# zhan-xu/MoRig

Measured on AMD Instinct MI355X. Metric: meshes/sec jointnet_motion forward, 4 k-vert synthetic, higher is better.
Workload: dtype f32 (split-fp16: 3x f16 MFMA, f32 accumulate); 1 GPU; jointnet_motion(num_keyframes=5, attn) eval forward, B=64 x 4096-vertex synthetic meshes/GPU, BASELINE.json configs[1]; step=COO->CSR prep + forward, meshes_per_gpu=64, global_batch=64, vertices_per_mesh=4096, parallelism=mesh-sharded dp1, guard_read=deferred, geo_graph=device

## Files before the change

include/morig_hip.h:

```cpp
#ifndef MORIG_HIP_H
#define MORIG_HIP_H

#include <stdint.h>
#include <string.h>

#ifdef __cplusplus
extern "C" {
#endif

#define MORIG_ABI_VERSION 3

#define MORIG_INIT_ARGS(type, var) type var; memset(&(var), 0, sizeof(var)); (var).struct_size = (uint32_t)sizeof(var)
#define MORIG_GEMM_ARGS_V3_SIZE        192u
#define MORIG_EDGECONV_ARGS_V3_SIZE    192u
#define MORIG_EDGECONV_X3_ARGS_V3_SIZE 168u
#define MORIG_SEGMAX_ARGS_V3_SIZE      144u
#define MORIG_POINTCONV_ARGS_V3_SIZE   176u
#define MORIG_EDGECONV_ARGS_SIZE       216u
#define MORIG_EDGECONV_X3_ARGS_SIZE    184u

#define MORIG_OK              0
#define MORIG_E_INVALID      -1
#define MORIG_E_UNSUPPORTED  -2
#define MORIG_E_HIP          -3
#define MORIG_E_NODEVICE     -4

int         morig_abi_version(void);
int         morig_reserve_cus(int n);
const char* morig_strerror(int status);
int         morig_last_hip_error(void);
int         morig_device_info(int* cu_count, int* lds_bytes_per_cu, int* clock_khz, char* arch, int arch_len);

int morig_csr_build(const int64_t* edge_index, int64_t n_edges, int32_t n_nodes,
                    int32_t* rowptr, int32_t* src_sorted, int32_t* dst_sorted,
                    int32_t* cursor, int32_t* status, void* stream);
#define MORIG_CSR_SKIP_NEGATIVE 1
#define MORIG_CSR_PAD4          2
#define MORIG_CSR_MIN4          4
int morig_csr_build_bipartite(const int64_t* edge_index, int64_t n_edges, int32_t n_src_nodes, int32_t n_nodes,
                              int32_t flags, int32_t* rowptr, int32_t* src_sorted, int32_t* dst_sorted,
                              int32_t* cursor, int32_t* status, void* stream);

#define MORIG_SPLIT_F16 0
#define MORIG_SPLIT_BF16 1
#define MORIG_SPLIT_BF16X6 2
typedef struct morig_gemm_args {
    uint32_t struct_size;
    int32_t M, N, K;
    const float* X; int32_t ldx;
    const float* W; int32_t ldw;
    const float* bias;
    const float* scale;
    const float* shift;
    int32_t relu;
    const float* rowbias; int32_t ld_rowbias;
    const int32_t* seg;
    float* Y; int32_t ldy;
    float* pool; int32_t ld_pool; int32_t n_seg;
    const void* W_split; int32_t* overflow;
    int32_t x_split, y_split;
    int32_t w_split_format;
    const float* X_tail; int32_t ld_tail, tail_rows, tail_cols;
} morig_gemm_args;
int morig_gemm(const morig_gemm_args* a, void* stream);

typedef struct morig_edgeconv_args {
    uint32_t struct_size;
    int32_t H;
    int32_t n_nodes, replicas;
    int32_t in_rep_stride;
    int32_t out_rep_stride;
    const float* A; int32_t lda;
    const float* B; int32_t ldb;
    const int32_t* rowptr; const int32_t* src_sorted; const int32_t* dst_sorted;
    int32_t edge_capacity;
    int32_t edge_count;
    const float* s1; const float* t1;
    const float* W2; int32_t ldw;
    const float* b2; const float* s2; const float* t2;
    float* out; int32_t ldo;
    const void* W2_split; int32_t* overflow;
    int32_t quad_aligned;
    int32_t out_split;
    int32_t exact_arith;
    int32_t seg_min4;
    const struct morig_edgeconv_args* init_with;
    const struct morig_edgeconv_args* split_with;
    int32_t skip_init, skip_split;
} morig_edgeconv_args;
int morig_edgeconv(const morig_edgeconv_args* a, void* stream);
int morig_edgeconv_can_split_out(const morig_edgeconv_args* a);

typedef struct morig_edgeconv_x3_args {
    uint32_t struct_size;
    int32_t H;
    int32_t n_nodes, replicas;
    int32_t in_rep_stride, out_rep_stride;
    const float* X; int32_t ldx;
    const float* W1a; const float* W1b; const float* b1;
    const int32_t* rowptr; const int32_t* src_sorted; const int32_t* dst_sorted;
    int32_t edge_capacity; int32_t edge_count;
    const float* W2; int32_t ldw;
    const float* b2; const float* s2; const float* t2;
    float* out; int32_t ldo;
    const void* W2_split; int32_t* overflow;
    const struct morig_edgeconv_x3_args* init_with;
    int32_t skip_init, reserved0;
} morig_edgeconv_x3_args;
int morig_edgeconv_x3(const morig_edgeconv_x3_args* a, void* stream);

int morig_edge_hidden(const morig_edgeconv_args* a, void* stream);
typedef struct morig_segmax_args {
    uint32_t struct_size;
    int32_t N, K;
    const float* X; int32_t ldx;
    const float* W; int32_t ldw;
    const float* bias; const float* scale; const float* shift; int32_t relu;
    const int32_t* rowptr; const int32_t* dst_sorted; int32_t n_nodes;
    int32_t edge_capacity; int32_t edge_count;
    float* out; int32_t ldo;
    const void* W_split; int32_t* overflow;
} morig_segmax_args;
int morig_segmax_gemm(const morig_segmax_args* a, void* stream);

typedef struct morig_pointconv_args {
    uint32_t struct_size;
    const float* A; int32_t lda;
    const float* B; int32_t ldb;
    const int64_t* slots; int32_t max_nbrs;
    int32_t n_centres, n_src;
    int32_t H, H3;
    const void* W2_split; int32_t ldw2; const float* b2;
    const void* W3_split; int32_t ldw3; const float* b3; const float* s3; const float* t3; int32_t relu3;
    float* out; int32_t ldo;
    int32_t* overflow; int32_t* status;
} morig_pointconv_args;
int morig_pointconv_fused(const morig_pointconv_args* a, void* stream);

int morig_copy2d(const float* src, int32_t lds, float* dst, int32_t ldd, int32_t rows, int32_t cols, void* stream);
int morig_copy2d_pad(const float* src, int32_t lds, int32_t rows, int32_t cols, float* dst, int32_t ldd,
                     int32_t slot_cols, int32_t split, int32_t* overflow, void* stream);
int morig_copy2d_pad_rep(const float* src, int32_t lds, int32_t rows, int32_t cols, int32_t src_col_step, float* dst,
                         int32_t ldd, int32_t slot_cols, int32_t replicas, int64_t dst_row_step, int32_t split,
                         int32_t* overflow, void* stream);
#define MORIG_MAX_TAILS 8
int morig_pack_tails(const float* src, int32_t lds, int32_t rows, const int32_t* col_a ,
                     const int32_t* col_b , int32_t wa, int32_t wb, int32_t n_tails, float* dst,
                     int64_t tail_stride, int32_t* overflow, void* stream);

int morig_gather_cols(const float* src, int32_t lds, const int32_t* cols, int32_t n_cols,
                      float* dst, int32_t ldd, int32_t rows, void* stream);

int morig_make_seg(const int64_t* batch, int32_t n_nodes, int32_t n_graphs, int32_t replicas,
                   int32_t* seg_out, void* stream);

int morig_rownorm(const float* x, int32_t ldx, int32_t rows_per_rep, int32_t replicas, int32_t cols,
                  float* y, int32_t ld_row, int32_t ld_rep, void* stream);

int morig_cls_attention(const float* x, int32_t n, int32_t T, int32_t C, int32_t heads,
                        const float* g, const float* cls, float* y, int32_t ldy, void* stream);

int morig_frame_reduce(const float* x, int32_t n, int32_t T, int32_t C, int32_t mode, float* y, int32_t ldy, void* stream);

int morig_csr_build_dual(const int64_t* edge_index, int64_t n_edges, int32_t n_nodes, int32_t* rowptr, int32_t* src_sorted,
                         int32_t* dst_sorted, int32_t* rowptr4, int32_t* src_sorted4, int32_t* dst_sorted4, int32_t* ws,
                         int32_t flags, int32_t* status, void* stream);
int morig_csr_from_slots(const int64_t* coo, int32_t n_nodes, int32_t max_nbrs, int32_t n_src_nodes,
                         int32_t* rowptr, int32_t* src_sorted, int32_t* dst_sorted, int32_t* cursor, int32_t* status,
                         void* stream);
int morig_fps(const float* pos, int32_t ldp, const int32_t* ptr, const int32_t* out_ptr, const int32_t* start,
              int32_t n_clouds, int32_t max_cloud_points, int32_t* idx_out, void* stream);
int morig_ball_query(const float* x, int32_t ldx, const int32_t* ptr_x, const float* y, int32_t ldy,
                     const int32_t* ptr_y, int32_t n_clouds, int32_t n_centres, float radius,
                     int32_t max_nbrs, int64_t* coo, void* stream);
int morig_radius_sample(const float* x, int32_t ldx, int32_t nx, const float* y, int32_t ldy, int32_t ny, float radius,
                        int32_t max_nbrs, uint32_t seed, int64_t* coo, int32_t* counts, void* stream);
int morig_knn_interpolate(const float* feat, int32_t ldf, int32_t C, const float* pos_x, int32_t ldx,
                          const int32_t* ptr_x, const float* pos_y, int32_t ldy, const int32_t* ptr_y,
                          int32_t n_clouds, int32_t n_targets, int32_t max_targets_per_cloud, int32_t k,
                          int32_t* idx_ws, float* wgt_ws, float* out, int32_t ldo, void* stream);
int morig_knn_search(const float* pos_x, int32_t ldx, const int32_t* ptr_x, const float* pos_y, int32_t ldy,
                     const int32_t* ptr_y, int32_t n_clouds, int32_t n_targets, int32_t max_targets_per_cloud, int32_t k,
                     int32_t* idx, float* wgt, void* stream);
int morig_knn_apply(const float* feat, int32_t ldf, int32_t C, const int32_t* idx, const float* wgt, int32_t n_targets,
                    float* out, int32_t ldo, void* stream);
int morig_cosine_nn(const float* v, int32_t ldv, const int32_t* ptr_v, const float* p, int32_t ldp,
                    const int32_t* ptr_p, int32_t n_clouds, int32_t max_rows_per_cloud, int32_t C,
                    int32_t* nn, float* sim, void* stream);
int morig_sigmoid_minmax(const float* x, int32_t ldx, const int32_t* ptr, int32_t n_meshes, float* out, int32_t ldo,
                         void* stream);
int morig_cosine_knn(const float* y, int32_t ldy, const int32_t* ptr_y, const float* x, int32_t ldx,
                     const int32_t* ptr_x, int32_t n_clouds, int32_t max_rows_per_cloud, int32_t C, int32_t k,
                     const float* vis, int32_t ld_vis, int32_t split, int32_t* idx, void* stream);
int morig_flow_vote(int32_t mode, const int32_t* idx, int32_t k, int32_t n, const float* feat_q, int32_t ldq,
                    const float* feat_s, int32_t lds, int32_t C, const float* pos_q, int32_t ldpq,
                    const float* pos_s, int32_t ldps, const float* vis, int32_t ld_vis, float* l1, int32_t ld_l1,
                    void* stream);
int morig_inside_check(const double* pts, int32_t n, const uint8_t* vox88, const double* translate, double scale,
                       double dims0, uint8_t* keep, void* stream);
int morig_knn_bandwidth(const double* pts, int32_t n, int32_t k, double* kth_ws, double* bandwidth, void* stream);
int morig_meanshift(const double* pts, const float* weights, int32_t n, const double* bandwidth, int32_t max_iter,
                    double* buf_a, double* buf_b, double* state, int32_t* result_in_a, void* stream);
int morig_nms_counts(const double* pts, int32_t n, const double* bandwidth, int32_t* counts, void* stream);
int morig_nms_greedy(const double* pts, const float* attn, int32_t n, const double* bandwidth, const int32_t* order,
                     double thrd_density, float thrd_attn, uint8_t* alive, void* stream);
int morig_knn_bandwidth_batched(const double* pts, const int32_t* ptr, int32_t n_meshes, int32_t n_all, int32_t max_n,
                                double quantile, double* kth_ws, double* bandwidth, void* stream);
int morig_meanshift_batched(const double* pts, const float* weights, const int32_t* ptr, int32_t n_meshes, int32_t n_all,
                            int32_t max_n, const double* bandwidth, int32_t max_iter, double* buf_a, double* buf_b,
                            double* state, int32_t* result_in_a, void* stream);
int morig_nms_counts_batched(const double* pts, const int32_t* ptr, int32_t n_meshes, int32_t n_all, int32_t max_n,
                             const double* bandwidth, int32_t* counts, void* stream);
int morig_nms_greedy_batched(const double* pts, const float* attn, const int32_t* ptr, int32_t n_meshes, int32_t n_all,
                             const double* bandwidth, const int32_t* order_local, double thrd_density, float thrd_attn,
                             uint8_t* alive, void* stream);
int morig_morton_keys(const double* pts, const int32_t* ptr, int32_t n_meshes, int32_t n_all, int64_t* keys, void* stream);
int morig_nms_counts_sorted(const double* pts, const int32_t* ptr, int32_t n_meshes, int32_t n_all, int32_t max_n,
                            const double* bandwidth, double* bbox_ws, int32_t* counts, void* stream);
int morig_meanshift_sorted(const double* pts, const float* weights, const int32_t* ptr, int32_t n_meshes, int32_t n_all,
                           int32_t max_n, const double* bandwidth, int32_t max_iter, double* buf_a, double* buf_b,
                           double* state, double* bbox_ws, int32_t* result_in_a, void* stream);
int morig_gather_rows(const float* src, int32_t lds, const int32_t* idx, int32_t rows, int32_t cols,
                      float* dst, int32_t ldd, void* stream);

int morig_geo_ball_graph(const float* pos, int32_t ldp, const int32_t* mesh_ptr, int32_t n_meshes, int32_t n_nodes,
                         float radius, int32_t max_nn, uint32_t seed, int32_t* slots, int32_t* counts, int32_t* members,
                         int32_t* offsets, int32_t* scan_ws, void* stream);
int morig_geo_ball_graph_dist(const double* dist, int64_t ldd, int32_t n_nodes, double radius, int32_t max_nn, uint32_t seed,
                              int32_t* slots, int32_t* counts, int32_t* members, int32_t* offsets, int32_t* scan_ws,
                              void* stream);
int morig_geo_ball_fill(const int32_t* slots, const int32_t* offsets, int32_t n_nodes, int32_t max_nn, int32_t self_loops,
                        int64_t* coo, int64_t n_out, void* stream);

int64_t morig_vol_geodesic_workspace(int32_t n_meshes, int32_t n_slots);
int morig_vol_geodesic(const uint8_t* vox, int32_t n_meshes, const double* vox_tf, const double* pos, const int32_t* vtx_ptr,
                       const double* bones, const int32_t* bone_ptr, int32_t n_jobs, const int64_t* dist_off, int32_t n_slots,
                       void* workspace, int64_t workspace_bytes, int32_t* status, int32_t* dist, void* stream);
int morig_skin_bind(const int32_t* dist, const int64_t* dist_off, const int32_t* vtx_ptr, const int32_t* bone_ptr, int32_t n_meshes,
                    int32_t n_vertices, const double* bones, const uint8_t* is_leaf, const int32_t* start_jid, const double* skins,
                    int32_t ld_skins, int32_t k, int32_t* bind_ids, double* bind_invd, double* labels, float* skin_input,
                    int64_t* skin_nn, int64_t* loss_mask, int64_t* skin_nnjids, void* stream);
int morig_skin_scatter(const float* logits, int32_t ldl, const int64_t* skin_nn, const int64_t* loss_mask, const int64_t* batch,
                       const int32_t* n_bones, int32_t n, int32_t k, int32_t mode, double* P, int32_t ldp, void* stream);
int morig_skin_filter(const double* P, int32_t ldp, const int32_t* rowptr, const int32_t* cols, const int64_t* batch,
                      const int32_t* n_bones, int32_t n, double ratio, double* W, int32_t ldw, void* stream);

int64_t morig_surface_geodesic_workspace(int64_t total_samples, int32_t n_meshes, int32_t max_samples, int32_t n_slots, int32_t use_lds);
int morig_surface_geodesic(const double* pts, const double* normals, const int32_t* s_ptr, const int32_t* job_ptr, int32_t n_meshes,
                           int64_t total_samples, int32_t max_samples, int32_t n_jobs, int32_t nsrc, int32_t use_lds,
                           const int64_t* out_off, int32_t n_slots, void* workspace, int64_t workspace_bytes, int32_t* status,
                           double* out, void* stream);
int morig_nearest_point(const double* q, const int32_t* q_ptr, const double* pts, const int32_t* p_ptr, int32_t n_meshes, int32_t n_q,
                        int32_t squared, int32_t* out, void* stream);
int morig_bone_point_distance(const double* pos, const int32_t* vtx_ptr, const double* bones, const int32_t* bone_ptr, int32_t n_meshes,
                              const int64_t* off, int64_t n_pairs, double* origins, double* dist, void* stream);
int morig_bone_visibility(const double* pos, const int32_t* vtx_ptr, const double* bones, const int32_t* bone_ptr, const double* tri_pos,
                          const int32_t* tp_ptr, const int32_t* faces, const int32_t* f_ptr, const int64_t* off, const int32_t* blk_ptr,
                          int32_t n_meshes, int32_t n_blocks, uint8_t* vis, void* stream);
int morig_bone_geodesic(const double* dist, const uint8_t* vis, const double* sg, const int64_t* sg_off, const int32_t* vtx_ptr,
                        const int32_t* bone_ptr, const int64_t* off, int32_t n_meshes, int32_t n_bones, int64_t n_pairs,
                        uint8_t* vis_after, int32_t* n_vis, double* pct, double* out, int32_t* nn, void* stream);
// ... 363 lines not shown
```

morig_amd/csrc/common.h:

```cpp
#pragma once
#include <hip/hip_runtime.h>
#include <stdint.h>
#include <string.h>
#include "../../include/morig_hip.h"
#include "ragged_core.h"
#include "mfma_types.h"
#include "launch_core.h"

namespace morig {

constexpr float FP16_RANGE_GUARD = 65000.f;

enum Kind : int {
    K_GEMM_BN128 = 0, K_GEMM_BN64, K_GEMM_BN32, K_GEMM_POOL,
    K_EDGE_H16, K_EDGE_H32, K_EDGE_H64, K_EDGE_H128, K_EDGE_H256,
    K_CSR, K_COPY, K_ROWNORM, K_ATTN, K_MISC,
    K_FPS, K_BALL, K_POINTCONV, K_KNN_INTERP, K_COSINE_NN,
    K_GEMM16_BN128, K_GEMM16_BN64, K_GEMM16_BN32, K_GEMM16_POOL,
    K_EDGE16_H32, K_EDGE16_H64, K_EDGE16_H128, K_EDGE16_H256, K_POINTCONV16, K_GEMM16_DMA,
    K_COSINE_KNN, K_FLOW_VOTE, K_JOINTS,
    K_GEMM16_DMAP, K_GEMM16_DMA128, K_EDGE16_H256_PP, K_EDGE16_H128_WS, K_EDGE16_PC, K_GEOGRAPH, K_EDGE16_X3, K_EDGE_X3, K_EDGE16_X3P, K_EDGE16_H128_RL,
    K_LOSS_NCE_FWD, K_LOSS_NCE_BWD, K_LOSS_MULTIPOS, K_LOSS_CHAMFER, K_LOSS_REDUCE,
    K_LOSS_LOGRATIO, K_LOSS_SKIN_CE,
    K_METRICS,
    K_RIG_ASSEMBLE, K_RIG_ENTRIES,
    K_RANSAC_VOTE, K_RANSAC_FIT, K_RANSAC_APPLY, K_KMEANS,
    K_MESH_PREP, K_VOXEL_SURFACE, K_VOXEL_FILL,
    K_POSE_PREP, K_POSE_SKIN, K_POSE_ERRORS,
    K_SCAN_RASTER, K_SCAN,
    K_SIMPLIFY_KEYS, K_SIMPLIFY_QUADRICS,
    K_RAY_CAST, K_RAY_SELECT, K_RAY_ATTENTION,
    K_TRANSFER_PAIRS, K_TRANSFER_FLOOD, K_TRANSFER_ROWS,
    K_BVH_BUILD, K_BVH_QUERY,
    K_COUNT
};
static_assert(K_COUNT <= MORIG_PROF_KINDS, "raise MORIG_PROF_KINDS");

void set_hip_error(hipError_t e);
struct ProfScope {
    ProfScope(int kind, hipStream_t s, double flops, double bytes);
    ~ProfScope();
    int slot; hipStream_t stream; ProfScope* outer;
};
void prof_retag(int kind);

inline int check_hip(hipError_t e) {
    if (e == hipSuccess) return MORIG_OK;
    set_hip_error(e);
    return MORIG_E_HIP;
}
#define MORIG_HIP_TRY(expr) do { hipError_t _e = (expr); if (_e != hipSuccess) { ::morig::set_hip_error(_e); return MORIG_E_HIP; } } while (0)
#define MORIG_LAUNCH_CHECK() MORIG_HIP_TRY(hipGetLastError())

struct EdgePcParams {
    int H;
    const float* W; int ldw;
    const float* bias; const float* scale; const float* shift;
    const float* A; int lda; const float* B; int ldb;
    const int* rowptr; const int* srcS; const int* dstS; int n_nodes; int rep_in; int rep_out; int tiles_per_rep;
    int replicas;
    float* Y; int ldy;
    int y16;
    int run;
    int* ovf;
    int quad;
    int min4;
    unsigned long long* trace;
    int dbg;
};
struct GemmDmaParams {
    int M, N, K;
    const float* X; int ldx;
    const float* Xt; int ldt; int tail_rows; int tail_chunks;
    const float* W; int ldw;
    const float* bias; const float* scale; const float* shift; int relu;
    const float* rowbias; int ld_rowbias; const int* seg;
    float* Y; int ldy; int y16;
    float* pool; int ld_pool;
    int tiles_n;
    int run;
    int* ovf;
    int dbg;
    unsigned long long* trace;
};
int launch_edge_pc(const EdgePcParams& p, int nblocks, hipStream_t s);
int launch_edge_pp(const EdgePcParams& p, int nblocks, hipStream_t s);
int launch_edge_ws(const EdgePcParams& p, int nblocks, hipStream_t s);
int launch_edge_rl(const EdgePcParams& p, int ntiles64, hipStream_t s);
int launch_gemm16_dma(const GemmDmaParams& p, int tiles_m128, hipStream_t s);
struct EdgeX3Params {
    const float* X; int ldx;
    const float* W1a; const float* W1b; const float* b1;
    const float* A; int lda; const float* B; int ldb;
    const float* W2s; int ldw;
    const float* bias; const float* scale; const float* shift;
    const int* rowptr; const int* srcS; const int* dstS; int n_nodes; int cap;
    int rep_in, rep_out, replicas;
    float* Y; int ldy;
    int* ovf;
};

int launch_edge_x3(const EdgeX3Params& p, int n_tiles_cap, hipStream_t s);
int launch_gemm16_dmap(const GemmDmaParams& p, hipStream_t s);
bool few_rows_gemm_takes(int M, int N, int K, int ldx, int ldw);
int launch_few_rows_gemm(const float* X, int ldx, int M, const float* W, int ldw, int N, int K, const float* bias, const float* scale,
                         const float* shift, int relu, float* Y, int ldy, hipStream_t s);

static_assert(sizeof(morig_gemm_args) >= MORIG_GEMM_ARGS_V3_SIZE && sizeof(morig_edgeconv_args) >= MORIG_EDGECONV_ARGS_V3_SIZE &&
              sizeof(morig_edgeconv_x3_args) >= MORIG_EDGECONV_X3_ARGS_V3_SIZE && sizeof(morig_segmax_args) >= MORIG_SEGMAX_ARGS_V3_SIZE &&
              sizeof(morig_pointconv_args) >= MORIG_POINTCONV_ARGS_V3_SIZE, "argument structs only grow");
static_assert(sizeof(morig_edgeconv_args) == MORIG_EDGECONV_ARGS_SIZE && sizeof(morig_edgeconv_x3_args) == MORIG_EDGECONV_X3_ARGS_SIZE,
              "include/morig_hip.h states the current sizes");
template <class T> static inline bool take_args(const T* a, T& mine, uint32_t v3_size) {
    if (!a) return false;
    const uint32_t n = a->struct_size;
    if (n < v3_size || n > 1024u || (n & 7u)) return false;
    memset(&mine, 0, sizeof(T));
    memcpy(&mine, a, n < sizeof(T) ? n : sizeof(T));
    mine.struct_size = (uint32_t)sizeof(T);
    return true;
}

static inline int cdiv(long a, long b) { return (int)((a + b - 1) / b); }

__device__ __forceinline__ void atomic_max_f32(float* addr, float v) {
    if (v == 0.0f) v = 0.0f;
    if (v >= 0.0f) atomicMax(reinterpret_cast<int*>(addr), __float_as_int(v));
    else           atomicMin(reinterpret_cast<unsigned int*>(addr), __float_as_uint(v));
}

__device__ __forceinline__ int xcd_remap(int b, int n) {
    const int q = n >> 3, r = n & 7, x = b & 7, i = b >> 3;
    return (x < r ? x * (q + 1) : r * (q + 1) + (x - r) * q) + i;
}

inline int stats_slab_rows(int rows_cap, int cols) {
    const int groups = (cols + 63) / 64;
    int slabs = 1024 / (groups > 0 ? groups : 1);
    if (slabs < 64) slabs = 64;
    int r = ((rows_cap > 0 ? rows_cap : 1) + slabs - 1) / slabs;
    r = (r + 3) & ~3;
    return r < 256 ? 256 : r;
}

#ifdef __HIPCC__
__device__ inline void split_pair_f16(float v0, float v1, float& hi, float& lo) {
    typedef __fp16 split_h2 __attribute__((ext_vector_type(2)));
    const split_h2 h = __builtin_amdgcn_cvt_pkrtz(v0, v1);
    hi = __builtin_bit_cast(float, h);
#ifdef MORIG_SPLIT_C_FORM
    split_h2 l;
    l[0] = (__fp16)(v0 - (float)h[0]); l[1] = (__fp16)(v1 - (float)h[1]);
    lo = __builtin_bit_cast(float, l);
#else
    asm("v_fma_mixlo_f16 %0, %1, 1.0, -%2 op_sel_hi:[0,0,1]" : "=v"(lo) : "v"(v0), "v"(hi));
    asm("v_fma_mixhi_f16 %0, %1, 1.0, -%2 op_sel:[0,0,1] op_sel_hi:[0,0,1]" : "+v"(lo) : "v"(v1), "v"(hi));
#endif
}
#endif

#ifdef __HIPCC__
__device__ inline void split_pair_bf16(float v0, float v1, float& hi, float& lo) {
    typedef __bf16 split_b2 __attribute__((ext_vector_type(2)));
    const split_b2 h = {(__bf16)v0, (__bf16)v1};
    const unsigned hb = __builtin_bit_cast(unsigned, h);
    hi = __builtin_bit_cast(float, h);
    const float r0 = v0 - __uint_as_float(hb << 16), r1 = v1 - __uint_as_float(hb & 0xffff0000u);
    const split_b2 l = {(__bf16)r0, (__bf16)r1};
    lo = __builtin_bit_cast(float, l);
}
#endif

#ifdef __HIPCC__
__device__ inline void split_pair_bf16_rem(float v0, float v1, float& hi, float& r0, float& r1) {
    typedef __bf16 split_b2 __attribute__((ext_vector_type(2)));
    const split_b2 h = {(__bf16)v0, (__bf16)v1};
    const unsigned hb = __builtin_bit_cast(unsigned, h);
    hi = __builtin_bit_cast(float, h);
    r0 = v0 - __uint_as_float(hb << 16);
    r1 = v1 - __uint_as_float(hb & 0xffff0000u);
}
#endif

template <int V> struct VecF { float v[V]; };
#ifdef __HIPCC__
template <int V> __device__ inline VecF<V> ldv(const float* p) {
    VecF<V> r;
    if constexpr (V == 4) { const float4 t = *reinterpret_cast<const float4*>(p); r.v[0] = t.x; r.v[1] = t.y; r.v[2] = t.z; r.v[3] = t.w; }
    else r.v[0] = *p;
    return r;
}
template <int V> __device__ inline void stv(float* p, const VecF<V>& r) {
    if constexpr (V == 4) *reinterpret_cast<float4*>(p) = make_float4(r.v[0], r.v[1], r.v[2], r.v[3]);
    else *p = r.v[0];
}
#endif
static inline bool vec4_ptr(const void* p, long ld) { return (reinterpret_cast<uintptr_t>(p) & 15) == 0 && (ld & 3) == 0; }

#ifdef __HIPCC__
__device__ inline void stats_block_store(const double (&acc)[2][4], int quads, int RL, int q, int rl, int c0, int cols, int slab,
                                         double* __restrict__ part) {
    __shared__ double sh[2 * 1024];
    const int gc = quads * 4;
    if (rl < RL) {
#pragma unroll
        for (int k = 0; k < 2; ++k)
#pragma unroll
            for (int j = 0; j < 4; ++j) sh[(k * gc + q * 4 + j) * RL + rl] = acc[k][j];
    }
    __syncthreads();
    const int t = threadIdx.x;
    if (t < 2 * gc) {
        const int k = t / gc, col = t - k * gc;
        double s = 0.0;
        for (int i = 0; i < RL; ++i) s += sh[(k * gc + col) * RL + i];
        if (c0 + col < cols) part[((size_t)slab * 2 + k) * cols + c0 + col] = s;
    }
}

constexpr int STATS_FC = 4;
__device__ inline void stats_final_sums(const double* __restrict__ part, int slabs, int cols, int c, double& s, double& q) {
    const int sl = threadIdx.x / STATS_FC, l = threadIdx.x % STATS_FC;
    constexpr int LANES = 256 / STATS_FC;
    s = 0.0; q = 0.0;
    if (c < cols)
        for (int b = sl; b < slabs; b += LANES) { s += part[((size_t)b * 2 + 0) * cols + c]; q += part[((size_t)b * 2 + 1) * cols + c]; }
    __shared__ double sh[2][LANES][STATS_FC];
    sh[0][sl][l] = s; sh[1][sl][l] = q;
    __syncthreads();
    for (int h = LANES / 2; h > 0; h >>= 1) {
        if (sl < h) { sh[0][sl][l] += sh[0][sl + h][l]; sh[1][sl][l] += sh[1][sl + h][l]; }
        __syncthreads();
    }
    s = sh[0][0][l]; q = sh[1][0][l];
}

__device__ __forceinline__ double block_sum256(double s, double* sh) {
    sh[threadIdx.x] = s;
    __syncthreads();
    for (int h = 128; h > 0; h >>= 1) {
        if ((int)threadIdx.x < h) sh[threadIdx.x] += sh[threadIdx.x + h];
        __syncthreads();
    }
    const double r = sh[0];
    __syncthreads();
    return r;
}
#endif

}
```

morig_amd/csrc/edge_x3.hip:

```cpp
#include "common.h"

namespace morig {


constexpr int X3_BM = 128, X3_LINE = 144;

template <bool AB>
__global__ __launch_bounds__(256, 4) void edge_x3_kernel(const EdgeX3Params p) {
    __shared__ __attribute__((aligned(16))) char lines[2][X3_BM * X3_LINE];
    __shared__ int sseg[2][X3_BM];
    __shared__ int sstart[2][X3_BM + 2];
    __shared__ int snseg[2];
    __shared__ int sflag[2][2];

    const int tid = threadIdx.x, lane = tid & 63, wave = tid >> 6;
    const int l31 = lane & 31, hi = lane >> 5;
    const int row = wave * 32 + l31;
    const int Etot = p.rowptr[p.n_nodes];
    const int tpr = (Etot + X3_BM - 1) / X3_BM;
    const int T = tpr * p.replicas;
    if ((int)blockIdx.x >= T) return;

    f16x8 w1h, w1l, wh[2], wl[2];
    {
        float v[8] = {0.f, 0.f, 0.f, 0.f, 0.f, 0.f, 0.f, 0.f};
        if (!AB && hi == 0) {
#pragma unroll
            for (int j = 0; j < 3; ++j) { v[j] = p.W1a[l31 * 4 + j]; v[3 + j] = p.W1b[l31 * 4 + j]; }
            v[6] = p.b1[l31];
        }
        f32x4 hb, lb;
#pragma unroll
        for (int q = 0; q < 4; ++q) { float h2, l2; split_pair_f16(v[2 * q], v[2 * q + 1], h2, l2); hb[q] = h2; lb[q] = l2; }
        w1h = __builtin_bit_cast(f16x8, hb); w1l = __builtin_bit_cast(f16x8, lb);
        const char* wr = reinterpret_cast<const char*>(p.W2s + (size_t)l31 * p.ldw);
#pragma unroll
        for (int st = 0; st < 2; ++st) {
            wh[st] = *reinterpret_cast<const f16x8*>(wr + 32 * st + 16 * hi);
            wl[st] = *reinterpret_cast<const f16x8*>(wr + 64 + 32 * st + 16 * hi);
        }
    }
    const float cb = p.bias[l31], cs = p.scale[l31], ct = p.shift[l31];

    auto tile_row0 = [&](int t, int& rep) __attribute__((always_inline)) { rep = t / tpr; return (t - rep * tpr) * X3_BM; };
    auto load_ids = [&](int t, int& d, int& sidx, int& edge) __attribute__((always_inline)) {
        if (t >= T) return;
        int rep; const int r0 = tile_row0(t, rep);
        const int r = min(r0 + row, Etot - 1);
        d = p.dstS[r]; sidx = p.srcS[r];
        if (tid < 2) edge = p.dstS[min(max(tid == 0 ? r0 - 1 : r0 + X3_BM, 0), Etot - 1)];
    };
    auto load_x = [&](int t, int d, int sidx, f32x4& a, f32x4& b) __attribute__((always_inline)) {
        if (AB || t >= T || hi != 0) return;
        int rep; const int r0 = tile_row0(t, rep);
        const bool live = r0 + row < Etot;
        const size_t base = (size_t)rep * p.rep_in;
        a = *reinterpret_cast<const f32x4*>(p.X + (base + (live ? d : 0)) * p.ldx);
        b = *reinterpret_cast<const f32x4*>(p.X + (base + (live ? sidx : 0)) * p.ldx);
    };
    auto load_ab = [&](int t, int d, int sidx, f32x4 (&a)[4], f32x4 (&b)[4]) __attribute__((always_inline)) {
        if (!AB || t >= T) return;
        int rep; const int r0 = tile_row0(t, rep);
        const bool live = r0 + row < Etot;
        const size_t base = (size_t)rep * p.rep_in;
        const float* ar = p.A + (base + (live ? d : 0)) * p.lda + 4 * hi;
        const float* br = p.B + (base + (live ? sidx : 0)) * p.ldb + 4 * hi;
#pragma unroll
        for (int g4 = 0; g4 < 4; ++g4) { a[g4] = *reinterpret_cast<const f32x4*>(ar + 8 * g4); b[g4] = *reinterpret_cast<const f32x4*>(br + 8 * g4); }
    };
    const int t0 = blockIdx.x, tstep = gridDim.x;
    int d_cur = 0, s_cur = 0, e_cur = 0, d_nxt = 0, s_nxt = 0, e_nxt = 0;
    f32x4 xi_cur = {0.f, 0.f, 0.f, 0.f}, xj_cur = xi_cur, xi_nxt = xi_cur, xj_nxt = xi_cur;
    f32x4 ga_cur[4], gb_cur[4], ga_nxt[4], gb_nxt[4];
#pragma unroll
    for (int g4 = 0; g4 < 4; ++g4) ga_cur[g4] = gb_cur[g4] = ga_nxt[g4] = gb_nxt[g4] = xi_cur;
    load_ids(t0, d_cur, s_cur, e_cur);
    load_ids(t0 + tstep, d_nxt, s_nxt, e_nxt);
    load_x(t0, d_cur, s_cur, xi_cur, xj_cur);
    load_ab(t0, d_cur, s_cur, ga_cur, gb_cur);
    bool amax_bad = false;

    int par = 0;
    for (int t = t0; t < T; t += tstep, par ^= 1) {
        int rep; const int r0 = tile_row0(t, rep);
        const bool live = r0 + row < Etot;
        load_x(t + tstep, d_nxt, s_nxt, xi_nxt, xj_nxt);
        load_ab(t + tstep, d_nxt, s_nxt, ga_nxt, gb_nxt);
        int d_nn = 0, s_nn = 0, e_nn = 0;
        load_ids(t + 2 * tstep, d_nn, s_nn, e_nn);

        char* L = lines[par];
        if (hi == 0) sseg[par][row] = live ? d_cur : -1;
        if (tid == 0) sflag[par][0] = (r0 > 0 && d_cur == e_cur) ? 1 : 0;
        {
            f32x16 a1;
            if constexpr (AB) {
#pragma unroll
                for (int g4 = 0; g4 < 4; ++g4)
#pragma unroll
                    for (int q = 0; q < 4; ++q) a1[4 * g4 + q] = ga_cur[g4][q] + gb_cur[g4][q];
            } else {
                f32x4 hb = {0.f, 0.f, 0.f, 0.f}, lb = hb;
                if (hi == 0) {
                    float h2, l2;
                    split_pair_f16(xi_cur[0], xi_cur[1], h2, l2); hb[0] = h2; lb[0] = l2;
                    split_pair_f16(xi_cur[2], xj_cur[0], h2, l2); hb[1] = h2; lb[1] = l2;
                    split_pair_f16(xj_cur[1], xj_cur[2], h2, l2); hb[2] = h2; lb[2] = l2;
                    split_pair_f16(1.0f, 0.0f, h2, l2);           hb[3] = h2; lb[3] = l2;
                    const float am = fmaxf(fmaxf(fmaxf(fabsf(xi_cur[0]), fabsf(xi_cur[1])), fmaxf(fabsf(xi_cur[2]), fabsf(xj_cur[0]))),
                                           fmaxf(fabsf(xj_cur[1]), fabsf(xj_cur[2])));
                    if (!(am < FP16_RANGE_GUARD)) amax_bad = true;
                }
                const f16x8 xh = __builtin_bit_cast(f16x8, hb), xl = __builtin_bit_cast(f16x8, lb);
#pragma unroll
                for (int r = 0; r < 16; ++r) a1[r] = 0.f;
                a1 = __builtin_amdgcn_mfma_f32_32x32x16_f16(w1l, xh, a1, 0, 0, 0);
                a1 = __builtin_amdgcn_mfma_f32_32x32x16_f16(w1h, xl, a1, 0, 0, 0);
                a1 = __builtin_amdgcn_mfma_f32_32x32x16_f16(w1h, xh, a1, 0, 0, 0);
            }
            char* line = L + row * X3_LINE;
            float am = 0.f, chk = 0.f;
#pragma unroll
            for (int g4 = 0; g4 < 4; ++g4) {
                float h[4];
#pragma unroll
                for (int q = 0; q < 4; ++q) {
                    if (AB) chk = fmaf(a1[4 * g4 + q], 0.f, chk);
                    h[q] = fmaxf(a1[4 * g4 + q], 0.f); am = fmaxf(am, h[q]);
                }
                float h0, l0, h1, l1;
                split_pair_f16(h[0], h[1], h0, l0);
                split_pair_f16(h[2], h[3], h1, l1);
                typedef float f32x2 __attribute__((ext_vector_type(2)));
                const f32x2 hv = {h0, h1}, lv = {l0, l1};
                const int c0 = 8 * g4 + 4 * hi;
                *reinterpret_cast<f32x2*>(line + 2 * c0) = hv;
                *reinterpret_cast<f32x2*>(line + 64 + 2 * c0) = lv;
            }
            if (!(chk == 0.f) || !(am < FP16_RANGE_GUARD)) amax_bad = true;
        }
        asm volatile("" ::: "memory");
        f32x16 acc;
#pragma unroll
        for (int r = 0; r < 16; ++r) acc[r] = 0.f;
        {
            const char* ar = L + (wave * 32 + l31) * X3_LINE + 16 * hi;
#pragma unroll
            for (int st = 0; st < 2; ++st) {
                const f16x8 ah = *reinterpret_cast<const f16x8*>(ar + 32 * st);
                const f16x8 al = *reinterpret_cast<const f16x8*>(ar + 64 + 32 * st);
                acc = __builtin_amdgcn_mfma_f32_32x32x16_f16(al, wh[st], acc, 0, 0, 0);
                acc = __builtin_amdgcn_mfma_f32_32x32x16_f16(ah, wl[st], acc, 0, 0, 0);
                acc = __builtin_amdgcn_mfma_f32_32x32x16_f16(ah, wh[st], acc, 0, 0, 0);
            }
        }
        asm volatile("" ::: "memory");
        {
            float* Z = reinterpret_cast<float*>(L);
#pragma unroll
            for (int r = 0; r < 16; ++r) {
                const int rl = wave * 32 + (r & 3) + 8 * (r >> 2) + 4 * hi;
                Z[rl * (X3_LINE / 4) + l31] = fmaxf(acc[r] + cb, 0.f) * cs + ct;
            }
        }
        __syncthreads();
        if (wave == 0) {
            const int rA = lane, rB = lane + 64;
            const bool f0 = rA == 0 || sseg[par][rA] != sseg[par][rA - 1];
            const bool f1 = sseg[par][rB] != sseg[par][rB - 1];
            const unsigned long long m0 = __ballot(f0), m1 = __ballot(f1);
            const unsigned long long below = (1ull << lane) - 1ull;
            if (f0) sstart[par][__popcll(m0 & below)] = rA;
            if (f1) sstart[par][__popcll(m0) + __popcll(m1 & below)] = rB;
            if (lane == 0) { const int ns = __popcll(m0) + __popcll(m1); snseg[par] = ns; sstart[par][ns] = X3_BM; }
            if (lane == 1) sflag[par][1] = (r0 + X3_BM < Etot && sseg[par][X3_BM - 1] == e_cur) ? 1 : 0;
        }
        __syncthreads();
        {
            const float* Z = reinterpret_cast<const float*>(L);
            const int c4 = (tid & 7) * 4, slot = tid >> 3;
            const int nseg = snseg[par];
            const bool first_cont = sflag[par][0] != 0, last_cont = sflag[par][1] != 0;
            float* obase = p.Y + (size_t)rep * p.rep_out * p.ldy + c4;
            for (int k = slot; k < nseg; k += 32) {
                const int rs = sstart[par][k], re = sstart[par][k + 1];
                const int sg = sseg[par][rs];
                if (sg < 0) continue;
                f32x4 m = *reinterpret_cast<const f32x4*>(Z + rs * (X3_LINE / 4) + c4);
                for (int r = rs + 1; r < re; r += 4) {
                    f32x4 z[4];
#pragma unroll
                    for (int u = 0; u < 4; ++u) z[u] = *reinterpret_cast<const f32x4*>(Z + min(r + u, re - 1) * (X3_LINE / 4) + c4);
#pragma unroll
                    for (int u = 0; u < 4; ++u)
#pragma unroll
                        for (int q = 0; q < 4; ++q) m[q] = fmaxf(m[q], z[u][q]);
                }
                float* o = obase + (size_t)sg * p.ldy;
                const bool partial = (rs == 0 && first_cont) || (re == X3_BM && last_cont);
                if (partial) {
#pragma unroll
                    for (int q = 0; q < 4; ++q) atomic_max_f32(o + q, m[q]);
                } else {
                    *reinterpret_cast<f32x4*>(o) = m;
                }
            }
        }
        d_cur = d_nxt; s_cur = s_nxt; e_cur = e_nxt; xi_cur = xi_nxt; xj_cur = xj_nxt;
        if constexpr (AB) {
#pragma unroll
            for (int g4 = 0; g4 < 4; ++g4) { ga_cur[g4] = ga_nxt[g4]; gb_cur[g4] = gb_nxt[g4]; }
        }
        d_nxt = d_nn; s_nxt = s_nn; e_nxt = e_nn;
    }
    if (amax_bad) *p.ovf = 1;
}

int launch_edge_x3(const EdgeX3Params& p, int n_tiles_cap, hipStream_t s) {
    int avail = cu_count() - reserved_cus();
    if (avail < 8) avail = 8;
    int grid = avail * 4;
    if (grid > n_tiles_cap) grid = n_tiles_cap;
    if (grid < 1) grid = 1;
    if (p.X) hipLaunchKernelGGL(edge_x3_kernel<false>, dim3(grid), dim3(256), 0, s, p);
    else     hipLaunchKernelGGL(edge_x3_kernel<true>, dim3(grid), dim3(256), 0, s, p);
    MORIG_LAUNCH_CHECK();
    return MORIG_OK;
}

}
```

morig_amd/csrc/prof.hip:

```cpp
#include "common.h"
#include <atomic>
#include <mutex>
#include <stdlib.h>
#include <vector>
#include <string.h>

namespace morig {

static int g_last_hip = 0;
void set_hip_error(hipError_t e) { g_last_hip = (int)e; }

int cu_count() {
    static std::atomic<int> cache[64];
    int dev = 0;
    if (hipGetDevice(&dev) != hipSuccess || dev < 0 || dev >= 64) return 256;
    int n = cache[dev].load();
    if (n == 0) {
        if (hipDeviceGetAttribute(&n, hipDeviceAttributeMultiprocessorCount, dev) != hipSuccess || n <= 0) n = 256;
        cache[dev].store(n);
    }
    return n;
}

static std::atomic<int> g_reserved_cus{0};
void set_reserved_cus(int n) { g_reserved_cus.store(n < 0 ? 0 : n); }
int reserved_cus() { return g_reserved_cus.load(); }

int persistent_grid(int units) {
    int ncu = cu_count();
    ncu = ncu > 8 ? (ncu / 8) * 8 : 8;
    int avail = ncu - ((reserved_cus() + 7) / 8) * 8;
    if (avail < 8) avail = 8;
    return units < avail ? ((units + 7) / 8) * 8 : avail;
}

int debug_flags() {
    static const int v = [] { const char* e = getenv("MORIG_DEBUG_FLAGS"); return e ? atoi(e) : 0; }();
    return v;
}

struct Slot { hipEvent_t a, b; int kind; double flops, bytes; };
static std::mutex g_mu;
static bool g_on = false;
static std::vector<Slot> g_slots;
static std::vector<Slot> g_free;
static double g_ms[K_COUNT], g_fl[K_COUNT], g_by[K_COUNT];
static long long g_n[K_COUNT];

static thread_local ProfScope* t_scope = nullptr;

ProfScope::ProfScope(int kind, hipStream_t s, double flops, double bytes) : slot(-1), stream(s), outer(t_scope) {
    t_scope = this;
    std::lock_guard<std::mutex> lk(g_mu);
    if (!g_on) return;
    Slot sl;
    if (!g_free.empty()) { sl = g_free.back(); g_free.pop_back(); }
    else {
        if (hipEventCreate(&sl.a) != hipSuccess) return;
        if (hipEventCreate(&sl.b) != hipSuccess) { (void)hipEventDestroy(sl.a); return; }
    }
    sl.kind = kind; sl.flops = flops; sl.bytes = bytes;
    (void)hipEventRecord(sl.a, s);
    g_slots.push_back(sl);
    slot = (int)g_slots.size() - 1;
}
ProfScope::~ProfScope() {
    t_scope = outer;
    if (slot < 0) return;
    std::lock_guard<std::mutex> lk(g_mu);
    if (slot < (int)g_slots.size()) (void)hipEventRecord(g_slots[slot].b, stream);
}

void prof_retag(int kind) {
    ProfScope* p = t_scope;
    if (!p || p->slot < 0) return;
    std::lock_guard<std::mutex> lk(g_mu);
    if (p->slot < (int)g_slots.size()) g_slots[p->slot].kind = kind;
}

static void drain_locked() {
    for (auto& s : g_slots) {
        float ms = 0.f;
        if (hipEventSynchronize(s.b) == hipSuccess && hipEventElapsedTime(&ms, s.a, s.b) == hipSuccess) {
            g_ms[s.kind] += ms; g_fl[s.kind] += s.flops; g_by[s.kind] += s.bytes; g_n[s.kind] += 1;
        }
        g_free.push_back(s);
    }
    g_slots.clear();
}

static const char* kNames[K_COUNT] = {
    "gemm_f32_bn128", "gemm_f32_bn64", "gemm_f32_bn32", "gemm_f32_pool",
    "edgeconv_h16", "edgeconv_h32", "edgeconv_h64", "edgeconv_h128", "edgeconv_h256",
    "csr_build", "copy", "rownorm", "cls_attention", "misc",
    "fps", "ball_query", "pointconv", "knn_interpolate", "cosine_nn",
    "gemm_f16x3_bn128", "gemm_f16x3_bn64", "gemm_f16x3_bn32", "gemm_f16x3_pool",
    "edgeconv_f16x3_h32", "edgeconv_f16x3_h64", "edgeconv_f16x3_h128", "edgeconv_f16x3_h256", "pointconv_f16x3", "gemm_f16x3_dma",
    "cosine_knn", "flow_vote", "joint_extraction",
    "gemm_f16x3_dmap", "gemm_f16x3_dma128", "edgeconv_f16x3_h256_pp", "edgeconv_f16x3_h128_ws", "edgeconv_f16x3_pc", "geo_graph", "edgeconv_f16x3_x3", "edgeconv_x3", "edgeconv_f16x3_x3_persistent", "edgeconv_f16x3_h128_rl",
    "loss_infonce_fwd", "loss_infonce_bwd", "loss_multipos", "loss_chamfer", "loss_reduce",
    "loss_logratio", "loss_skin_ce",
    "rig_metrics",
    "rig_assemble", "rig_skin_entries",
    "ransac_vote", "ransac_fit", "ransac_apply", "kernel_kmeans",
    "mesh_prep", "voxel_surface", "voxel_fill",
    "pose_prep", "pose_skin", "pose_traj_errors",
    "scan_raster", "scan",
    "simplify_keys", "simplify_quadrics",
    "ray_cast", "ray_select", "ray_attention",
    "transfer_pairs", "transfer_flood", "transfer_rows",
    "bvh_build", "bvh_query",
};
static const char* kSymbols[K_COUNT] = {
    "tile_kernel<128, 32, 0, 0, 0,", "tile_kernel<64, 32, 0, 0, 0,", "tile_kernel<32, 32, 0, 0, 0,", "tile_kernel<128, 32, 0, 1, 0,",
    "tile_kernel<32, 16, 1, 2, 0,", "tile_kernel<32, 32, 1, 2, 0,", "tile_kernel<64, 32, 1, 2, 0,", "tile_kernel<128, 32, 1, 2, 0,", "tile_kernel<256, 16, 1, 2, 0,",
    nullptr, nullptr, "rownorm", "cls_attention_kernel", nullptr,
    nullptr, nullptr, nullptr, nullptr, nullptr,
    "tile_kernel<128, 32, 0, 0, 1,", "tile_kernel<64, 32, 0, 0, 1,", "tile_kernel<32, 32, 0, 0, 1,", "gemm16_dmap_kernel<true>",
    "tile_kernel<32, 32, 1, 2, 1,", "tile_kernel<64, 32, 1, 2, 1,", "edge_pp_kernel<128", "edge_ws_kernel<256", nullptr, "gemm16_dma_kernel<256, 256, 4, 2",
    nullptr, nullptr, nullptr,
    "gemm16_dmap_kernel<false>", "gemm16_dma_kernel<128, 128, 2, 2", "edge_pp_kernel<256", "edge_ws_kernel<128", "edge_pc_kernel", "geo_ball_graph_kernel", "tile_kernel<32, 32, 2, 2, 1,", "tile_kernel<32, 32, 2, 2, 0,", "edge_x3_kernel", "edge_rl128_kernel",
    "nce_fwd_kernel", "nce_bwd_kernel", nullptr, nullptr, nullptr,
    nullptr, nullptr,
    nullptr,
    "rig_assemble_kernel", nullptr,
    "ransac_vote_kernel", "ransac_fit_kernel", "ransac_apply_kernel", "kmeans_kernel",
    nullptr, "voxel_surface_kernel", "voxel_fill_kernel",
    nullptr, "pose_skin_kernel", "pose_errors_kernel",
    nullptr, nullptr,
    nullptr, "simplify_quadrics_kernel",
    "ray_cast_kernel", "ray_select_kernel", "ray_attention_kernel",
    nullptr, nullptr, nullptr,
    nullptr, nullptr,
};

}

using namespace morig;

extern "C" {

int morig_abi_version(void) { return MORIG_ABI_VERSION; }

int morig_reserve_cus(int n) { set_reserved_cus(n); return MORIG_OK; }

const char* morig_strerror(int st) {
    switch (st) {
        case MORIG_OK: return "ok";
        case MORIG_E_INVALID: return "invalid argument (null pointer, negative size or misaligned leading dimension)";
        case MORIG_E_UNSUPPORTED: return "unsupported width/shape for the instantiated gfx950 kernels";
        case MORIG_E_HIP: return "HIP runtime error (see morig_last_hip_error)";
        case MORIG_E_NODEVICE: return "no gfx950 device visible";
        default: return "unknown status";
    }
}

int morig_last_hip_error(void) { return g_last_hip; }

int morig_device_info(int* cu_count, int* lds_bytes_per_cu, int* clock_khz, char* arch, int arch_len) {
    int n = 0;
    if (hipGetDeviceCount(&n) != hipSuccess || n <= 0) return MORIG_E_NODEVICE;
    int dev = 0;
    MORIG_HIP_TRY(hipGetDevice(&dev));
    hipDeviceProp_t p;
    MORIG_HIP_TRY(hipGetDeviceProperties(&p, dev));
    if (cu_count) *cu_count = p.multiProcessorCount;
    if (lds_bytes_per_cu) *lds_bytes_per_cu = (int)p.maxSharedMemoryPerMultiProcessor;
    if (clock_khz) *clock_khz = p.clockRate;
    if (arch && arch_len > 0) { strncpy(arch, p.gcnArchName, arch_len - 1); arch[arch_len - 1] = 0; }
    return strncmp(p.gcnArchName, "gfx950", 6) == 0 ? MORIG_OK : MORIG_E_NODEVICE;
}

int morig_prof_enable(int on) {
    std::lock_guard<std::mutex> lk(g_mu);
    int prev = g_on ? 1 : 0;
    g_on = on != 0;
    return prev;
}

int morig_prof_reset(void) {
    std::lock_guard<std::mutex> lk(g_mu);
    drain_locked();
    for (int k = 0; k < K_COUNT; ++k) { g_ms[k] = g_fl[k] = g_by[k] = 0.0; g_n[k] = 0; }
    return MORIG_OK;
}

const char* morig_prof_name(int kind) { return (kind >= 0 && kind < K_COUNT) ? kNames[kind] : nullptr; }
const char* morig_prof_symbol(int kind) { return (kind >= 0 && kind < K_COUNT) ? kSymbols[kind] : nullptr; }

int morig_prof_collect(int kind, int64_t* launches, double* total_ms, double* flops, double* bytes) {
    if (kind < 0 || kind >= K_COUNT) return MORIG_E_INVALID;
    std::lock_guard<std::mutex> lk(g_mu);
    drain_locked();
    if (launches) *launches = g_n[kind];
    if (total_ms) *total_ms = g_ms[kind];
    if (flops) *flops = g_fl[kind];
    if (bytes) *bytes = g_by[kind];
    return MORIG_OK;
}

}
```

morig_amd/csrc/tile_gemm.hip:

```cpp
#include "common.h"
#include "epilogue_store.h"
#include <stdint.h>
#include <stdlib.h>
#include <type_traits>

namespace morig {

typedef _Float16 f16x4 __attribute__((ext_vector_type(4)));
typedef __fp16 f16x2 __attribute__((ext_vector_type(2)));

enum { PREC_F32 = 0, PREC_F16X3 = 1, PREC_BF16X3 = 2, PREC_BF16X6 = 3 };

enum { LOAD_DENSE = 0, LOAD_EDGE = 1, LOAD_EDGE3 = 2 };
enum { MODE_STORE = 0, MODE_POOL = 1, MODE_EDGEMAX = 2 };

struct TileParams {
    int M, N, K;
    const float* W; int ldw;
    const float* bias; const float* scale; const float* shift; int relu;
    const float* X; int ldx;
    const float* A; int lda; const float* B; int ldb;
    const float* X3; int ldx3; const float* W1a; const float* W1b; const float* b1;
    const int* rowptr; const int* srcS; const int* dstS; int n_nodes; int rep_in; int rep_out; int tiles_per_rep;
    const float* s1; const float* t1;
// ... 392 lines not shown
        }
        __syncthreads();
        const int c4 = (tid & 7) * 4, slot = tid >> 3;
        const int col0 = tn * BN + c4;
        if (col0 >= p.N) return;
        const int nseg = snseg;
        float* obase = p.Y + (size_t)rep * p.rep_out * p.ldy + col0;
        const bool vec_ok = (reinterpret_cast<uintptr_t>(p.Y) & 15) == 0 && (p.ldy & 3) == 0 && col0 + 4 <= p.N;
        for (int k = slot; k < nseg; k += 32) {
            const int rs = sstart[k], re = sstart[k + 1];
            const int sg = sseg[rs];
            if (sg < 0) continue;
            f32x4 m = *reinterpret_cast<const f32x4*>(Z + rs * ZL + c4);
            for (int r = rs + 1; r < re; r += 4) {
                f32x4 z[4];
#pragma unroll
                for (int u = 0; u < 4; ++u) z[u] = *reinterpret_cast<const f32x4*>(Z + min(r + u, re - 1) * ZL + c4);
#pragma unroll
                for (int u = 0; u < 4; ++u)
#pragma unroll
                    for (int q = 0; q < 4; ++q) m[q] = fmaxf(m[q], z[u][q]);
            }
            float* o = obase + (size_t)sg * p.ldy;
            const bool partial = (rs == 0 && first_cont) || (re == BM && last_cont);
            if (partial) {
#pragma unroll
                for (int q = 0; q < 4; ++q) if (col0 + q < p.N) atomic_max_f32(o + q, m[q]);
            } else if (vec_ok) {
                *reinterpret_cast<f32x4*>(o) = m;
            } else {
#pragma unroll
                for (int q = 0; q < 4; ++q) if (col0 + q < p.N) o[q] = m[q];
            }
        }
        return;
    }
    constexpr int NTP = ((ZC / 32) / WN) >= 1 ? ((ZC / 32) / WN) : 1;
    constexpr int NPASS = NT / NTP;
    static_assert(NTP * WN * 32 == ZC && NPASS * NTP == NT, "epilogue column blocking");
    constexpr int G = 256 / ZC;
    constexpr int RG = BM / G;
    const int zc = tid % ZC, zg = tid / ZC;
    const int r0 = (ZC == 64) ? __builtin_amdgcn_readfirstlane(zg * RG) : zg * RG;
    unsigned long long seg_start_lo = 0, seg_start_hi = 0, seg_own = 0; int seg_id_own = 0;
    if constexpr (MODE == MODE_EDGEMAX && ZC == 64) {
        const int s_lo = sseg[lane], s_hi = sseg[lane + 64];
        const int p_lo = sseg[lane > 0 ? lane - 1 : 0], p_hi = sseg[lane + 63];
        seg_start_lo = __ballot(lane == 0 || s_lo != p_lo); seg_start_hi = __ballot(s_hi != p_hi);
        const bool up = r0 >= 64;
        const unsigned long long valid = up ? __ballot(s_hi >= 0) : __ballot(s_lo >= 0);
        seg_own = (up ? seg_start_hi : seg_start_lo) & valid & (((1ull << RG) - 1ull) << (r0 & 63));
        seg_id_own = up ? s_hi : s_lo;
    }
    auto run_pass = [&](auto cb_const) {
        constexpr int cb = decltype(cb_const)::value;
        __syncthreads();
#pragma unroll
        for (int j = 0; j < NTP; ++j) {
            constexpr int dummy = 0; (void)dummy;
            const int nt = cb * NTP + j;
            const int col = tn * BN + wn * NT * 32 + nt * 32 + l31;
            const float b = (p.bias && col < p.N) ? p.bias[col] : 0.f;
            const float sc = (p.scale && col < p.N) ? p.scale[col] : 1.f;
            const float sh = (p.shift && col < p.N) ? p.shift[col] : 0.f;
#pragma unroll
            for (int mt = 0; mt < MT; ++mt)
#pragma unroll
                for (int r = 0; r < 16; ++r) {
                    const int rl = wm * MT * 32 + mt * 32 + (r & 3) + 8 * (r >> 2) + 4 * hi;
                    float v = acc[mt][nt][r] + b;
                    if (p.relu) v = v > 0.f ? v : 0.f;
                    Z[rl * ZLD + (wn * NTP + j) * 32 + l31] = v * sc + sh;
                }
        }
        __syncthreads();
        const int wz = zc / (NTP * 32), jz = (zc >> 5) % NTP;
        const int col = tn * BN + wz * NT * 32 + (cb * NTP + jz) * 32 + (zc & 31);
        if (col >= p.N) return;
        const float* zcolp = Z + zc;
        if (MODE == MODE_POOL) {
            int cur = -2; bool open = false; float m = 0.f;
#pragma unroll
            for (int bt = 0; bt < RG / 16; ++bt) {
                const int rb0 = r0 + bt * 16;
                float zv[16]; int sv[16];
#pragma unroll
                for (int i = 0; i < 16; ++i) {
                    sv[i] = (ZC == 64) ? __builtin_amdgcn_readfirstlane(sseg[rb0 + i]) : sseg[rb0 + i];
                    zv[i] = zcolp[(rb0 + i) * ZLD];
                }
#pragma unroll
                for (int i = 0; i < 16; ++i) {
                    if (sv[i] != cur) {
                        if (open) atomic_max_f32(p.Y + (size_t)cur * p.ldy + col, m);
                        cur = sv[i]; open = cur >= 0; m = zv[i];
                    } else if (open) m = fmaxf(m, zv[i]);
                }
            }
            if (open) atomic_max_f32(p.Y + (size_t)cur * p.ldy + col, m);
        } else {
            if constexpr (ZC == 64) {
            float* obase = p.Y + (size_t)rep * p.rep_out * p.ldy + col;
            const bool upper = r0 >= 64;
            unsigned long long mine = seg_own;
            while (mine) {
                const int bl = __builtin_ctzll(mine);
                mine &= mine - 1ull;
                const unsigned long long above = bl < 63 ? ~((2ull << bl) - 1ull) : 0ull;
                int rs, re;
                if (upper) {
                    const unsigned long long later = seg_start_hi & above;
                    rs = 64 + bl; re = later ? 64 + __builtin_ctzll(later) : BM;
                } else {
                    const unsigned long long later = seg_start_lo & above;
                    rs = bl; re = later ? __builtin_ctzll(later) : (seg_start_hi ? 64 + __builtin_ctzll(seg_start_hi) : BM);
                }
                const int sg = __builtin_amdgcn_readlane(seg_id_own, bl);
                float m = zcolp[rs * ZLD];
                for (int r = rs + 1; r < re; r += 4) {
                    const int l = re - 1;
                    const float z0 = zcolp[r * ZLD], z1 = zcolp[min(r + 1, l) * ZLD], z2 = zcolp[min(r + 2, l) * ZLD], z3 = zcolp[min(r + 3, l) * ZLD];
                    m = fmaxf(fmaxf(m, z0), fmaxf(fmaxf(z1, z2), z3));
                }
                float* o = obase + (size_t)sg * p.ldy;
                if ((rs == 0 && first_cont) || (re == BM && last_cont)) atomic_max_f32(o, m); else *o = m;
            }
            }
        }
    };
    run_pass(std::integral_constant<int, 0>{});
    if constexpr (NPASS > 1) run_pass(std::integral_constant<int, 1>{});
    if constexpr (NPASS > 2) run_pass(std::integral_constant<int, 2>{});
    if constexpr (NPASS > 3) run_pass(std::integral_constant<int, 3>{});
    static_assert(NPASS <= 4, "column passes");
}

__device__ __forceinline__ int straddled_row(const int* __restrict__ rowptr, const int* __restrict__ dstS, int n_nodes, int tile_rows,
                                             int run, int replicas, int rep_out, int g, int n_cand, bool last_only) {
    if (g > n_cand) return -1;
    const int Etot = rowptr[n_nodes];
    const int tpr = (Etot + tile_rows - 1) / tile_rows;
    if (tpr <= 0) return -1;
    const long long t = (long long)g * run;
    const int rep = (int)(t / tpr), tile = (int)(t - (long long)rep * tpr);
    if (rep >= replicas || tile == 0) return -1;
    const int e = tile * tile_rows;
    const int d = dstS[e];
    if (rowptr[d] >= e) return -1;
    if (last_only && (long long)e + (long long)run * tile_rows < rowptr[d + 1]) return -1;
    return rep * rep_out + d;
}

struct BoundaryJob { const int* rowptr; const int* dstS; int n_nodes, H; float* out; int ldo, rep_out, tile_rows, run, replicas, n_cand; int* ovf; };
struct BoundaryJobs { BoundaryJob j[2]; };

__global__ __launch_bounds__(256) void init_boundary_rows_kernel(const BoundaryJobs js) {
    const BoundaryJob& b = js.j[blockIdx.y];
    if ((int)blockIdx.x * 256 >= b.n_cand) return;
    const int* __restrict__ rowptr = b.rowptr; const int* __restrict__ dstS = b.dstS;
    float* __restrict__ out = b.out;
    const int H = b.H, ldo = b.ldo;
    const int lane = threadIdx.x & 63;
    const int d = straddled_row(rowptr, dstS, b.n_nodes, b.tile_rows, b.run, b.replicas, b.rep_out, blockIdx.x * 256 + threadIdx.x + 1, b.n_cand, false);
    const bool vec = ((reinterpret_cast<uintptr_t>(out) | (uintptr_t)(ldo * 4) | (uintptr_t)(H * 4)) & 15) == 0;
    typedef unsigned u32x4 __attribute__((ext_vector_type(4)));
    unsigned long long todo = __ballot(d >= 0);
    while (todo) {
        const int l = __builtin_ctzll(todo);
        todo &= todo - 1;
        float* orow = out + (size_t)__builtin_amdgcn_readlane(d, l) * ldo;
        if (vec) {
            u32x4* o4 = reinterpret_cast<u32x4*>(orow);
            for (int c = lane; c < H / 4; c += 64) o4[c] = u32x4{0xFFFFFFFFu, 0xFFFFFFFFu, 0xFFFFFFFFu, 0xFFFFFFFFu};
        } else {
            unsigned* o = reinterpret_cast<unsigned*>(orow);
            for (int c = lane; c < H; c += 64) o[c] = 0xFFFFFFFFu;
        }
    }
}

static BoundaryJob boundary_job(const int* rowptr, const int* dstS, int n_nodes, int edge_capacity, int H, float* out, int ldo, int rep_out,
                                int slots, int tile_rows, int run, int* ovf) {
    BoundaryJob b = {};
    b.rowptr = rowptr; b.dstS = dstS; b.n_nodes = n_nodes; b.H = H; b.out = out; b.ldo = ldo; b.rep_out = rep_out;
    b.tile_rows = tile_rows; b.run = run; b.replicas = slots; b.ovf = ovf;
    const int n_cand = cdiv((long)cdiv(edge_capacity, tile_rows) * slots, run) - 1;
    b.n_cand = n_cand > 0 ? n_cand : 0;
    return b;
}

static int init_boundary_rows(const BoundaryJob* jobs, int n, hipStream_t s) {
    BoundaryJobs js = {};
    int m = 0, most = 0;
    for (int i = 0; i < n; ++i) if (jobs[i].n_cand > 0) { js.j[m++] = jobs[i]; most = jobs[i].n_cand > most ? jobs[i].n_cand : most; }
    if (m == 0) return MORIG_OK;
    hipLaunchKernelGGL(init_boundary_rows_kernel, dim3(cdiv(most, 256), m), dim3(256), 0, s, js);
    MORIG_LAUNCH_CHECK();
    return MORIG_OK;
}

static int init_boundary_rows(const int* rowptr, const int* dstS, int n_nodes, int edge_capacity, int H, float* out, int ldo,
                              int rep_out, int slots, hipStream_t s, int tile_rows = 128, int run = 1) {
    const BoundaryJob b = boundary_job(rowptr, dstS, n_nodes, edge_capacity, H, out, ldo, rep_out, slots, tile_rows, run, nullptr);
    return init_boundary_rows(&b, 1, s);
}

__global__ __launch_bounds__(256) void split_boundary_rows_kernel(const BoundaryJobs js) {
    const BoundaryJob& b = js.j[blockIdx.y];
    if ((int)blockIdx.x * 64 >= b.n_cand) return;
    const int* __restrict__ rowptr = b.rowptr; const int* __restrict__ dstS = b.dstS;
    float* __restrict__ out = b.out;
    int* __restrict__ ovf = b.ovf;
    const int H = b.H, ldo = b.ldo;
    const int lane = threadIdx.x & 63;
    const int g = (blockIdx.x * 4 + (threadIdx.x >> 6)) * 16 + lane + 1;
    const int d = lane < 16 ? straddled_row(rowptr, dstS, b.n_nodes, b.tile_rows, b.run, b.replicas, b.rep_out, g, b.n_cand, true) : -1;
    unsigned long long todo = __ballot(d >= 0);
    float am = 0.f;
    bool bad = false;
    while (todo) {
        int dr[4];
#pragma unroll
        for (int i = 0; i < 4; ++i) {
            const int l = todo ? __builtin_ctzll(todo) : -1;
            todo &= todo - 1;
            dr[i] = l >= 0 ? __builtin_amdgcn_readlane(d, l) : -1;
        }
        for (int c0 = 0; c0 < H; c0 += 256) {
            const int c = c0 + 4 * lane;
            float4 v[4];
#pragma unroll
            for (int i = 0; i < 4; ++i)
                if (dr[i] >= 0 && c < H) v[i] = *reinterpret_cast<const float4*>(out + (size_t)dr[i] * ldo + c);
#pragma unroll
            for (int i = 0; i < 4; ++i)
                if (dr[i] >= 0 && c < H) {
                    float h0, l0, h1, l1;
                    split_pair_f16(v[i].x, v[i].y, h0, l0);
                    split_pair_f16(v[i].z, v[i].w, h1, l1);
                    am = fmaxf(am, fmaxf(fmaxf(fabsf(v[i].x), fabsf(v[i].y)), fmaxf(fabsf(v[i].z), fabsf(v[i].w))));
                    bad |= !(v[i].x == v[i].x && v[i].y == v[i].y && v[i].z == v[i].z && v[i].w == v[i].w);
                    char* oc = reinterpret_cast<char*>(out + (size_t)dr[i] * ldo) + (c >> 5) * 128 + (c & 31) * 2;
                    *reinterpret_cast<float2*>(oc) = make_float2(h0, h1);
                    *reinterpret_cast<float2*>(oc + 64) = make_float2(l0, l1);
                }
        }
    }
    if (bad || !(am < FP16_RANGE_GUARD)) *ovf = 1;
}

static int split_boundary_rows(const BoundaryJob* jobs, int n, hipStream_t s) {
    BoundaryJobs js = {};
    int m = 0, most = 0;
    for (int i = 0; i < n; ++i) if (jobs[i].n_cand > 0) { js.j[m++] = jobs[i]; most = jobs[i].n_cand > most ? jobs[i].n_cand : most; }
    if (m == 0) return MORIG_OK;
    hipLaunchKernelGGL(split_boundary_rows_kernel, dim3(cdiv(most, 64), m), dim3(256), 0, s, js);
    MORIG_LAUNCH_CHECK();
    return MORIG_OK;
}

template <int BN, int KC, int LOAD, int MODE, int PREC = PREC_F32>
static int launch_tile(const TileParams& p0, int nblocks, hipStream_t s) {
    TileParams p = p0;
    p.dbg = debug_flags();
    if constexpr (BN == 128 && KC == 32 && LOAD == LOAD_DENSE && MODE == MODE_STORE) {
        static const bool no_fast = getenv("MORIG_TILE_NO_FAST") != nullptr;
        if (p.dbg == 0 && !no_fast && p.M % 128 == 0 && p.K % KC == 0) {
            hipLaunchKernelGGL((tile_kernel<BN, KC, LOAD, MODE, PREC, true>), dim3(nblocks), dim3(256), 0, s, p);
            MORIG_LAUNCH_CHECK();
            return MORIG_OK;
        }
    }
    hipLaunchKernelGGL((tile_kernel<BN, KC, LOAD, MODE, PREC>), dim3(nblocks), dim3(256), 0, s, p);
    MORIG_LAUNCH_CHECK();
    return MORIG_OK;
}

static inline bool aligned16(const void* p) { return (reinterpret_cast<uintptr_t>(p) & 15) == 0; }

__global__ void pool_identity_to_zero_kernel(float* __restrict__ pool, int64_t n) {
    const int64_t stride = (int64_t)gridDim.x * blockDim.x;
    unsigned* u = reinterpret_cast<unsigned*>(pool);
    for (int64_t i = (int64_t)blockIdx.x * blockDim.x + threadIdx.x; i < n; i += stride) if (u[i] == 0xFFFFFFFFu) u[i] = 0u;
}
static int pool_finalize(float* pool, int n_seg, int ld_pool, hipStream_t s) {
    const int64_t n = (int64_t)n_seg * ld_pool;
    int64_t blocks = (n + 255) / 256;
    if (blocks > 1024) blocks = 1024;
    hipLaunchKernelGGL(pool_identity_to_zero_kernel, dim3((int)blocks), dim3(256), 0, s, pool, n);
    MORIG_LAUNCH_CHECK();
    return MORIG_OK;
}

}

using namespace morig;

extern "C" int morig_gemm(const morig_gemm_args* a_in, void* stream) {
    morig_gemm_args mine;
    if (!take_args(a_in, mine, MORIG_GEMM_ARGS_V3_SIZE)) return MORIG_E_INVALID;
    const morig_gemm_args* a = &mine;
    if (!a->X || !a->W) return MORIG_E_INVALID;
    if (a->M < 0 || a->N <= 0 || a->K <= 0) return MORIG_E_INVALID;
    if (a->M == 0) return MORIG_OK;
    if ((a->ldx & 3) || (a->ldw & 3) || !aligned16(a->X) || !aligned16(a->W)) return MORIG_E_INVALID;
    const bool tail = a->X_tail != nullptr;
    if (tail) {
        if (!a->x_split || !a->W_split || a->tail_cols <= 0 || (a->tail_cols & 31) || (a->K & 31) || a->K <= a->tail_cols || a->tail_rows <= 0 ||
            (a->ld_tail & 31) || a->ld_tail < a->tail_cols || (reinterpret_cast<uintptr_t>(a->X_tail) & 127) ||
            (double)a->tail_rows * a->ld_tail * 4.0 >= 4.0e9) return MORIG_E_INVALID;
    }
    if (a->ldx < (((a->K - (tail ? a->tail_cols : 0)) + 3) & ~3) || a->ldw < ((a->K + 31) & ~31)) return MORIG_E_INVALID;
    const bool pool = a->pool != nullptr;
    if (tail && pool) return MORIG_E_UNSUPPORTED;
    if (!pool && !a->Y) return MORIG_E_INVALID;
    if (pool && a->Y) return MORIG_E_UNSUPPORTED;
    if ((pool || a->rowbias) && !a->seg) return MORIG_E_INVALID;
    hipStream_t s = reinterpret_cast<hipStream_t>(stream);

    TileParams p = {};
    p.M = a->M; p.N = a->N; p.K = a->K;
    p.W = a->W; p.ldw = a->ldw;
    p.bias = a->bias; p.scale = a->scale; p.shift = a->shift; p.relu = a->relu;
    p.X = a->X; p.ldx = a->ldx;
    p.rowbias = a->rowbias; p.ld_rowbias = a->ld_rowbias; p.seg = a->seg;
    const int tiles_m = cdiv(a->M, 128);
    const double flops = 2.0 * a->M * (double)a->N * a->K;
    const double bytes = 4.0 * ((double)a->M * a->K + (double)a->N * a->K + (pool ? 0.0 : (double)a->M * a->N));

    const bool x6 = a->W_split == nullptr && a->w_split_format == MORIG_SPLIT_BF16X6;
    if (x6 && (a->x_split || a->y_split)) return MORIG_E_INVALID;
    const bool f16 = a->W_split != nullptr;
    if (f16 && a->w_split_format != MORIG_SPLIT_F16 && a->w_split_format != MORIG_SPLIT_BF16) return MORIG_E_INVALID;
    const bool bf16 = f16 && a->w_split_format == MORIG_SPLIT_BF16;
    if (f16 && !bf16 && a->overflow == nullptr) return MORIG_E_INVALID;
    if (f16) {
        if (!aligned16(a->W_split)) return MORIG_E_INVALID;
        if (bf16 && (pool || a->x_split || a->y_split)) return MORIG_E_UNSUPPORTED;
        p.W = static_cast<const float*>(a->W_split); p.ovf = a->overflow;
    }
    const bool kc64 = f16 && a->K >= 64 && (a->ldw & 63) == 0 && a->ldw >= ((a->K + 63) & ~63) && !getenv("MORIG_KC32");
    if (a->x_split || a->y_split) {
        if (!f16) return MORIG_E_INVALID;
        if (a->x_split && ((a->ldx & 31) || a->ldx < (((a->K - (tail ? a->tail_cols : 0)) + 31) & ~31) || (reinterpret_cast<uintptr_t>(a->X) & 127))) return MORIG_E_INVALID;
        if (a->y_split && (pool || (a->ldy & 31) || (reinterpret_cast<uintptr_t>(a->Y) & 127))) return MORIG_E_INVALID;
        p.x16 = a->x_split ? 1 : 0; p.y16 = a->y_split ? 1 : 0;
    }
    if (pool) {
        if (a->n_seg <= 0 || a->ld_pool < a->N) return MORIG_E_INVALID;
        MORIG_HIP_TRY(hipMemsetAsync(a->pool, 0xFF, (size_t)a->n_seg * a->ld_pool * sizeof(float), s));
        if (f16 && a->x_split && a->N > 64 && !getenv("MORIG_NO_DMA")) {
            GemmDmaParams q = {};
            q.M = a->M; q.N = a->N; q.K = a->K; q.X = a->X; q.ldx = a->ldx; q.W = p.W; q.ldw = p.ldw;
            q.bias = a->bias; q.scale = a->scale; q.shift = a->shift; q.relu = a->relu; q.seg = a->seg;
            q.pool = a->pool; q.ld_pool = a->ld_pool; q.ovf = a->overflow;
            ProfScope ps(K_GEMM16_POOL, s, flops, bytes);
            const int st = launch_gemm16_dma(q, tiles_m, s);
            return st != MORIG_OK ? st : pool_finalize(a->pool, a->n_seg, a->ld_pool, s);
        }
        p.Y = a->pool; p.ldy = a->ld_pool;
        p.tiles_n = cdiv(a->N, 128);
        ProfScope ps(f16 ? K_GEMM16_POOL : K_GEMM_POOL, s, flops, bytes);
        int st;
        if (x6) st = launch_tile<128, 32, LOAD_DENSE, MODE_POOL, PREC_BF16X6>(p, tiles_m * p.tiles_n, s);
        else if (f16 && kc64 && getenv("MORIG_KC64")) st = launch_tile<128, 64, LOAD_DENSE, MODE_POOL, PREC_F16X3>(p, tiles_m * p.tiles_n, s);
        else st = f16 ? launch_tile<128, 32, LOAD_DENSE, MODE_POOL, PREC_F16X3>(p, tiles_m * p.tiles_n, s)
                      : launch_tile<128, 32, LOAD_DENSE, MODE_POOL>(p, tiles_m * p.tiles_n, s);
        return st != MORIG_OK ? st : pool_finalize(a->pool, a->n_seg, a->ld_pool, s);
    }
    p.Y = a->Y; p.ldy = a->ldy;
    if (f16 && a->x_split && a->N > 64 && !getenv("MORIG_NO_DMA")) {
        GemmDmaParams q = {};
        q.M = a->M; q.N = a->N; q.K = a->K; q.X = a->X; q.ldx = a->ldx; q.W = p.W; q.ldw = p.ldw;
        q.bias = a->bias; q.scale = a->scale; q.shift = a->shift; q.relu = a->relu;
        q.rowbias = a->rowbias; q.ld_rowbias = a->ld_rowbias; q.seg = a->seg;
        q.Y = a->Y; q.ldy = a->ldy; q.y16 = a->y_split ? 1 : 0; q.tiles_n = cdiv(a->N, 128); q.ovf = a->overflow;
        if (tail) { q.Xt = a->X_tail; q.ldt = a->ld_tail; q.tail_rows = a->tail_rows; q.tail_chunks = a->tail_cols / 32; }
        ProfScope ps(K_GEMM16_DMA, s, flops, bytes);
        return launch_gemm16_dma(q, tiles_m, s);
    }
    if (tail) return MORIG_E_UNSUPPORTED;
    if (!bf16 && !a->rowbias && !a->x_split && !a->y_split && few_rows_gemm_takes(a->M, a->N, a->K, a->ldx, a->ldw)) {
        ProfScope ps(K_MISC, s, flops, bytes);
        return launch_few_rows_gemm(a->X, a->ldx, a->M, a->W, a->ldw, a->N, a->K, a->bias, a->scale, a->shift, a->relu, a->Y, a->ldy, s);
    }
    if (bf16) {
        ProfScope ps(K_MISC, s, flops, bytes);
        if (a->N > 64) { p.tiles_n = cdiv(a->N, 128); return launch_tile<128, 32, LOAD_DENSE, MODE_STORE, PREC_BF16X3>(p, tiles_m * p.tiles_n, s); }
        p.tiles_n = 1;
        if (a->N > 32) return launch_tile<64, 32, LOAD_DENSE, MODE_STORE, PREC_BF16X3>(p, tiles_m, s);
        return launch_tile<32, 32, LOAD_DENSE, MODE_STORE, PREC_BF16X3>(p, tiles_m, s);
    }
    if (x6) {
        ProfScope ps(a->N > 64 ? K_GEMM_BN128 : (a->N > 32 ? K_GEMM_BN64 : K_GEMM_BN32), s, flops, bytes);
        if (a->N > 64) { p.tiles_n = cdiv(a->N, 128); return launch_tile<128, 32, LOAD_DENSE, MODE_STORE, PREC_BF16X6>(p, tiles_m * p.tiles_n, s); }
        p.tiles_n = 1;
        if (a->N > 32) return launch_tile<64, 32, LOAD_DENSE, MODE_STORE, PREC_BF16X6>(p, tiles_m, s);
        return launch_tile<32, 32, LOAD_DENSE, MODE_STORE, PREC_BF16X6>(p, tiles_m, s);
    }
    if (a->N > 64) {
        p.tiles_n = cdiv(a->N, 128);
        ProfScope ps(f16 ? K_GEMM16_BN128 : K_GEMM_BN128, s, flops, bytes);
        static const bool want64 = getenv("MORIG_KC64") != nullptr;
        if (f16 && kc64 && want64) return launch_tile<128, 64, LOAD_DENSE, MODE_STORE, PREC_F16X3>(p, tiles_m * p.tiles_n, s);
        return f16 ? launch_tile<128, 32, LOAD_DENSE, MODE_STORE, PREC_F16X3>(p, tiles_m * p.tiles_n, s)
                   : launch_tile<128, 32, LOAD_DENSE, MODE_STORE>(p, tiles_m * p.tiles_n, s);
// ... 126 lines not shown
    static const bool want_mix = [] { const char* e = getenv("MORIG_EDGE_MIX"); return !(e && e[0] == '0'); }();
    pl.mix = pl.wide && !one_shot && !want_pp && pl.pp_ok && !a->quad_aligned && a->seg_min4 && a->H == 256 && want_mix &&
             (a->lda & 3) == 0 && (a->ldb & 3) == 0;
    pl.use_ws = (quad_ok && !pl.use_rl && (a->H == 256 || ws128)) || (pl.mix && a->out_split);
    pl.tile_rows = ((pl.use_ws && a->H == 256) || pl.use_rl) ? 64 : 128;
    static const int run_env = [] { const char* e = getenv("MORIG_EDGE_RUN"); const int v = e ? atoi(e) : 8; return v < 1 ? 1 : (v > 4096 ? 4096 : v); }();
    pl.run = 1;
    if (pl.use_rl || (pl.use_ws && a->out_split)) {
        const long tiles = (long)cdiv(a->edge_capacity, pl.tile_rows) * a->replicas;
        const long units = pl.use_rl ? 2048 : 256;
        while (pl.run * 2 <= run_env && tiles / (units * 16) >= pl.run * 2) pl.run *= 2;
    }
    static const bool no_split = [] { const char* e = getenv("MORIG_EDGE_SPLIT_OUT"); return e && e[0] == '0'; }();
    pl.split_ok = (pl.use_rl || pl.use_ws || pl.mix) && !no_split && a->overflow != nullptr && (a->ldo & 31) == 0 &&
                  (reinterpret_cast<uintptr_t>(a->out) & 127) == 0;
    return pl;
}

extern "C" int morig_edgeconv_can_split_out(const morig_edgeconv_args* a_in) {
    morig_edgeconv_args mine;
    if (!take_args(a_in, mine, MORIG_EDGECONV_ARGS_V3_SIZE)) return 0;
    const morig_edgeconv_args* a = &mine;
    TileParams p = {};
    if (edge_common(a, p) != MORIG_OK) return 0;
    return edge_plan(a).split_ok ? 1 : 0;
}

extern "C" int morig_edgeconv(const morig_edgeconv_args* a_in, void* stream) {
    morig_edgeconv_args mine;
    if (!take_args(a_in, mine, MORIG_EDGECONV_ARGS_V3_SIZE)) return MORIG_E_INVALID;
    const morig_edgeconv_args* a = &mine;
    TileParams p = {};
    const int st = edge_common(a, p);
    if (st != MORIG_OK) return st;
    if (a->in_rep_stride < 0 || (a->replicas > 1 && a->out_rep_stride < a->n_nodes)) return MORIG_E_INVALID;
    hipStream_t s = reinterpret_cast<hipStream_t>(stream);
    const int nblocks = p.tiles_per_rep * a->replicas;
    const bool f16 = a->W2_split != nullptr;
    const EdgePlan pl = edge_plan(a);
    const bool wide = pl.wide, one_shot = pl.one_shot, pp_ok = pl.pp_ok, use_rl = pl.use_rl, use_ws = pl.use_ws;
    if (a->out_split && !pl.split_ok) return MORIG_E_UNSUPPORTED;

    auto job_of = [](const morig_edgeconv_args* q, const EdgePlan& qp) {
        return boundary_job(q->rowptr, q->dst_sorted, q->n_nodes, q->edge_capacity, q->H, q->out, q->ldo, q->out_rep_stride, q->replicas,
                            qp.tile_rows, qp.run, q->overflow);
    };
    morig_edgeconv_args other;
    auto partner = [&](const morig_edgeconv_args* q_in, EdgePlan& qp) -> int {
        if (!take_args(q_in, other, MORIG_EDGECONV_ARGS_V3_SIZE)) return MORIG_E_INVALID;
        TileParams tp = {};
        const int stp = edge_common(&other, tp);
        if (stp != MORIG_OK) return stp;
        if (other.in_rep_stride < 0 || (other.replicas > 1 && other.out_rep_stride < other.n_nodes)) return MORIG_E_INVALID;
        qp = edge_plan(&other);
        if (other.out_split && !qp.split_ok) return MORIG_E_UNSUPPORTED;
        return MORIG_OK;
    };
    if (!a->skip_init) {
        BoundaryJob jobs[2];
        int nj = 0;
        jobs[nj++] = job_of(a, pl);
        if (a->init_with) {
            EdgePlan qp;
            const int stp = partner(a->init_with, qp);
            if (stp != MORIG_OK) return stp;
            jobs[nj++] = job_of(&other, qp);
        }
        const int st2 = init_boundary_rows(jobs, nj, s);
        if (st2 != MORIG_OK) return st2;
    } else if (a->init_with) return MORIG_E_INVALID;

    const double E = (double)(a->edge_count > 0 ? a->edge_count : a->edge_capacity) * a->replicas;
    const double flops = 2.0 * E * a->H * (double)a->H;
    const double bytes = 4.0 * a->H * (double)a->n_nodes * (2.0 * (a->in_rep_stride > 0 ? a->replicas : 1) + a->replicas);
    if (wide) {
        EdgePcParams q = {};
        q.H = a->H; q.W = p.W; q.ldw = p.ldw; q.bias = p.bias; q.scale = p.scale; q.shift = p.shift;
        q.A = p.A; q.lda = p.lda; q.B = p.B; q.ldb = p.ldb;
        q.rowptr = p.rowptr; q.srcS = p.srcS; q.dstS = p.dstS; q.n_nodes = p.n_nodes;
        q.rep_in = p.rep_in; q.rep_out = p.rep_out; q.tiles_per_rep = p.tiles_per_rep; q.replicas = a->replicas;
        q.Y = p.Y; q.ldy = p.ldy; q.ovf = p.ovf; q.quad = a->quad_aligned ? 1 : 0; q.min4 = a->seg_min4 ? 1 : 0;
        q.y16 = a->out_split ? 1 : 0; q.run = pl.run;
        ProfScope ps(a->H == 256 ? K_EDGE16_H256 : K_EDGE16_H128, s, flops, bytes);
        if (use_rl || use_ws) {
            int st3;
            if (use_rl) {
                prof_retag(K_EDGE16_H128_RL);
                st3 = launch_edge_rl(q, cdiv(a->edge_capacity, 64) * a->replicas, s);
            } else {
                if (a->H == 128) prof_retag(K_EDGE16_H128_WS);
                st3 = launch_edge_ws(q, cdiv(a->edge_capacity, a->H == 256 ? 64 : 128) * a->replicas, s);
            }
            if (st3 != MORIG_OK || !a->out_split) return (st3 == MORIG_OK && (a->split_with || a->skip_split)) ? MORIG_E_INVALID : st3;
            if (a->skip_split) return a->split_with ? MORIG_E_INVALID : MORIG_OK;
            BoundaryJob jobs[2];
            int nj = 0;
            jobs[nj++] = job_of(a, pl);
            if (a->split_with) {
                EdgePlan qp;
                const int stp = partner(a->split_with, qp);
                if (stp != MORIG_OK) return stp;
                if (!other.out_split || !(qp.use_rl || qp.use_ws)) return MORIG_E_INVALID;
                jobs[nj++] = job_of(&other, qp);
            }
            return split_boundary_rows(jobs, nj, s);
        }
        if (a->split_with || a->skip_split) return MORIG_E_INVALID;
        if (one_shot || !pp_ok) { prof_retag(K_EDGE16_PC); return launch_edge_pc(q, nblocks, s); }
        if (a->H == 256) prof_retag(K_EDGE16_H256_PP);
        return launch_edge_pp(q, nblocks, s);
    }
    if (a->split_with || a->skip_split) return MORIG_E_INVALID;
    static const bool x3_tile = [] { const char* e = getenv("MORIG_X3_TILE"); return e && e[0] == '1'; }();
    if (f16 && a->H == 32 && !a->s1 && !x3_tile && (a->ldo & 3) == 0 && aligned16(a->out) && (a->lda & 3) == 0 && (a->ldb & 3) == 0 &&
        aligned16(a->b2) && a->ldw >= 32) {
        EdgeX3Params q = {};
        q.A = a->A; q.lda = a->lda; q.B = a->B; q.ldb = a->ldb;
        q.W2s = static_cast<const float*>(a->W2_split); q.ldw = a->ldw;
        q.bias = a->b2; q.scale = a->s2; q.shift = a->t2;
        q.rowptr = a->rowptr; q.srcS = a->src_sorted; q.dstS = a->dst_sorted; q.n_nodes = a->n_nodes; q.cap = a->edge_capacity;
        q.rep_in = a->in_rep_stride; q.rep_out = a->out_rep_stride; q.replicas = a->replicas;
        q.Y = a->out; q.ldy = a->ldo; q.ovf = a->overflow;
        ProfScope ps(K_EDGE16_H32, s, flops, bytes);
        return launch_edge_x3(q, nblocks, s);
    }
    if (f16) {
        switch (a->H) {
            case 32:  { ProfScope ps(K_EDGE16_H32, s, flops, bytes);  return launch_tile<32, 32, LOAD_EDGE, MODE_EDGEMAX, PREC_F16X3>(p, nblocks, s); }
            case 64:  { ProfScope ps(K_EDGE16_H64, s, flops, bytes);  return launch_tile<64, 32, LOAD_EDGE, MODE_EDGEMAX, PREC_F16X3>(p, nblocks, s); }
            case 128: { ProfScope ps(K_EDGE16_H128, s, flops, bytes); return launch_tile<128, 32, LOAD_EDGE, MODE_EDGEMAX, PREC_F16X3>(p, nblocks, s); }
            case 256: { ProfScope ps(K_EDGE16_H256, s, flops, bytes); return launch_tile<256, 32, LOAD_EDGE, MODE_EDGEMAX, PREC_F16X3>(p, nblocks, s); }
            default: return MORIG_E_UNSUPPORTED;
        }
    }
    if (a->exact_arith == 1) {
        switch (a->H) {
            case 32:  { ProfScope ps(K_EDGE_H32, s, flops, bytes);  return launch_tile<32, 32, LOAD_EDGE, MODE_EDGEMAX, PREC_BF16X6>(p, nblocks, s); }
            case 64:  { ProfScope ps(K_EDGE_H64, s, flops, bytes);  return launch_tile<64, 32, LOAD_EDGE, MODE_EDGEMAX, PREC_BF16X6>(p, nblocks, s); }
            case 128: { ProfScope ps(K_EDGE_H128, s, flops, bytes); return launch_tile<128, 32, LOAD_EDGE, MODE_EDGEMAX, PREC_BF16X6>(p, nblocks, s); }
            case 256: { ProfScope ps(K_EDGE_H256, s, flops, bytes); return launch_tile<256, 32, LOAD_EDGE, MODE_EDGEMAX, PREC_BF16X6>(p, nblocks, s); }
            default: break;
        }
    }
    switch (a->H) {
        case 16:  { ProfScope ps(K_EDGE_H16, s, flops, bytes);  return launch_tile<32, 16, LOAD_EDGE, MODE_EDGEMAX>(p, nblocks, s); }
        case 32:  { ProfScope ps(K_EDGE_H32, s, flops, bytes);  return launch_tile<32, 32, LOAD_EDGE, MODE_EDGEMAX>(p, nblocks, s); }
        case 64:  { ProfScope ps(K_EDGE_H64, s, flops, bytes);  return launch_tile<64, 32, LOAD_EDGE, MODE_EDGEMAX>(p, nblocks, s); }
        case 128: { ProfScope ps(K_EDGE_H128, s, flops, bytes); return launch_tile<128, 32, LOAD_EDGE, MODE_EDGEMAX>(p, nblocks, s); }
        case 256: { ProfScope ps(K_EDGE_H256, s, flops, bytes); return launch_tile<256, 16, LOAD_EDGE, MODE_EDGEMAX>(p, nblocks, s); }
        default: return MORIG_E_UNSUPPORTED;
    }
}

extern "C" int morig_edgeconv_x3(const morig_edgeconv_x3_args* a_in, void* stream) {
    morig_edgeconv_x3_args mine;
    if (!take_args(a_in, mine, MORIG_EDGECONV_X3_ARGS_V3_SIZE)) return MORIG_E_INVALID;
    const morig_edgeconv_x3_args* a = &mine;
    if (!a->X || !a->W1a || !a->W1b || !a->b1 || !a->rowptr || !a->src_sorted || !a->dst_sorted || !a->W2 || !a->out) return MORIG_E_INVALID;
    if (!a->b2 || !a->s2 || !a->t2) return MORIG_E_INVALID;
    if (a->H != 32) return MORIG_E_UNSUPPORTED;
    if (a->n_nodes <= 0 || a->replicas <= 0 || a->edge_capacity <= 0 || a->ldx < 4 || (a->ldx & 3) || !aligned16(a->X)) return MORIG_E_INVALID;
    if ((a->ldw & 3) || a->ldw < 32 || a->ldo < 32 || !aligned16(a->W2) || !aligned16(a->W1a) || !aligned16(a->W1b)) return MORIG_E_INVALID;
    if (a->in_rep_stride < 0 || (a->replicas > 1 && a->out_rep_stride < a->n_nodes)) return MORIG_E_INVALID;
    hipStream_t s = reinterpret_cast<hipStream_t>(stream);
    TileParams p = {};
    p.M = a->edge_capacity; p.N = 32; p.K = 32;
    p.W = a->W2; p.ldw = a->ldw;
    p.bias = a->b2; p.scale = a->s2; p.shift = a->t2; p.relu = 1;
    p.X3 = a->X; p.ldx3 = a->ldx; p.W1a = a->W1a; p.W1b = a->W1b; p.b1 = a->b1;
    p.rowptr = a->rowptr; p.srcS = a->src_sorted; p.dstS = a->dst_sorted;
    p.n_nodes = a->n_nodes; p.rep_in = a->in_rep_stride; p.rep_out = a->out_rep_stride;
    p.Y = a->out; p.ldy = a->ldo;
    p.tiles_per_rep = cdiv(a->edge_capacity, 128);
    p.tiles_n = 1;
    const bool f16 = a->W2_split != nullptr;
    if (f16) {
        if (!a->overflow || !aligned16(a->W2_split)) return MORIG_E_INVALID;
        p.W = static_cast<const float*>(a->W2_split); p.ovf = a->overflow;
    }
    const int nblocks = p.tiles_per_rep * a->replicas;
    if (!a->skip_init) {
        BoundaryJob jobs[2];
        int nj = 0;
        jobs[nj++] = boundary_job(a->rowptr, a->dst_sorted, a->n_nodes, a->edge_capacity, 32, a->out, a->ldo, a->out_rep_stride, a->replicas, 128, 1, nullptr);
        if (a->init_with) {
            morig_edgeconv_x3_args o;
            if (!take_args(a->init_with, o, MORIG_EDGECONV_X3_ARGS_V3_SIZE)) return MORIG_E_INVALID;
            if (!o.rowptr || !o.dst_sorted || !o.out || o.H != 32 || o.n_nodes <= 0 || o.replicas <= 0 || o.edge_capacity <= 0 || o.ldo < 32 ||
                (o.replicas > 1 && o.out_rep_stride < o.n_nodes)) return MORIG_E_INVALID;
            jobs[nj++] = boundary_job(o.rowptr, o.dst_sorted, o.n_nodes, o.edge_capacity, 32, o.out, o.ldo, o.out_rep_stride, o.replicas, 128, 1, nullptr);
        }
        const int st2 = init_boundary_rows(jobs, nj, s);
        if (st2 != MORIG_OK) return st2;
    } else if (a->init_with) return MORIG_E_INVALID;
    const double E = (double)(a->edge_count > 0 ? a->edge_count : a->edge_capacity) * a->replicas;
    ProfScope ps(f16 ? K_EDGE16_X3 : K_EDGE_X3, s, E * (2.0 * 32 * 32 + 12.0 * 32), 32.0 * E);
    static const bool want_tile = [] { const char* e = getenv("MORIG_X3_TILE"); return e && e[0] == '1'; }();
    if (f16 && !want_tile && (a->ldo & 3) == 0 && aligned16(a->out)) {
        EdgeX3Params q = {};
        q.X = a->X; q.ldx = a->ldx; q.W1a = a->W1a; q.W1b = a->W1b; q.b1 = a->b1;
        q.W2s = static_cast<const float*>(a->W2_split); q.ldw = a->ldw;
        q.bias = a->b2; q.scale = a->s2; q.shift = a->t2;
        q.rowptr = a->rowptr; q.srcS = a->src_sorted; q.dstS = a->dst_sorted; q.n_nodes = a->n_nodes; q.cap = a->edge_capacity;
        q.rep_in = a->in_rep_stride; q.rep_out = a->out_rep_stride; q.replicas = a->replicas;
        q.Y = a->out; q.ldy = a->ldo; q.ovf = a->overflow;
        prof_retag(K_EDGE16_X3P);
        return launch_edge_x3(q, nblocks, s);
    }
    return f16 ? launch_tile<32, 32, LOAD_EDGE3, MODE_EDGEMAX, PREC_F16X3>(p, nblocks, s)
               : launch_tile<32, 32, LOAD_EDGE3, MODE_EDGEMAX>(p, nblocks, s);
}
```

morig_amd/models/basic_modules.py:

```python
from __future__ import annotations

import itertools
import math
import os
import threading
from typing import Optional

import torch
from torch.nn import BatchNorm1d as BN, Linear as Lin, ReLU, Sequential as Seq

from .. import packing
from ..native import Mat
from ..runtime import get_ops

__all__ = ["MLP", "EdgeConv", "GCU", "EdgeConvMotion", "GCUMotion", "NativeModule"]


def MLP(channels, batch_norm=True):
    if not batch_norm:
        return Seq(*[Seq(Lin(a, b), ReLU()) for a, b in zip(channels[:-1], channels[1:])])
    return Seq(*[Seq(Lin(a, b), ReLU(), BN(b, momentum=0.1)) for a, b in zip(channels[:-1], channels[1:])])


def _invalidate_packed(module, incompatible_keys):
# ... 243 lines not shown

class GCU(NativeModule):

    def __init__(self, in_channels, out_channels, aggr="max"):
        super().__init__()
        self.edge_conv_tpl = EdgeConv(nn_pos=MLP([in_channels * 2, out_channels // 2, out_channels // 2]), aggr=aggr)
        self.edge_conv_geo = EdgeConv(nn_pos=MLP([in_channels * 2, out_channels // 2, out_channels // 2]), aggr=aggr)
        self.mlp = MLP([out_channels, out_channels])

    def _pack(self):
        vertex, (et, eg) = packing.pack_edge_pair([self.edge_conv_tpl.nn_pos, self.edge_conv_geo.nn_pos])
        return dict(vertex=vertex, et=et, eg=eg, mlp=packing.pack_mlp_layer(self.mlp[0]))

    def run(self, ops, x: Mat, csr_tpl, csr_geo, out: Mat, split_in: bool = False, split_out: bool = False):
        pk = self.packed(x.base.device)
        n, H = x.rows, pk["et"].H
        dev = x.base.device
        ab = ops.empty(n, 4 * H, dev)
        ops.gemm(x, pk["vertex"], relu=False, Y=Mat.of(ab), x_split=split_in)
        ec = ops.empty(n, 2 * H, dev)
        sp = H % 32 == 0 and _edge_rows_can_split(ops, ab, ec, csr_tpl, csr_geo, pk["et"], pk["eg"], H, 1, 0)
        ops.edgeconv_pair(dict(A=Mat.of(ab, 0, H), B=Mat.of(ab, H, H), csr=csr_tpl, ec=pk["et"], out=Mat.of(ec, 0, H), out_split=sp),
                          dict(A=Mat.of(ab, 2 * H, H), B=Mat.of(ab, 3 * H, H), csr=csr_geo, ec=pk["eg"], out=Mat.of(ec, H, H), out_split=sp))
        ops.gemm(Mat.of(ec), pk["mlp"], relu=True, Y=out, x_split=sp, y_split=split_out)

    def _forward(self, pos, tpl_edge_index, geo_edge_index):
        ops = get_ops()
        x = _padded_copy(ops, _as_matrix(pos))
        n = x.shape[0]
        pk = self.packed(x.device)
        out = ops.empty(n, pk["mlp"].N, x.device)
        self.run(ops, Mat.of(x, 0, pk["vertex"].K), ops.csr_build(tpl_edge_index, n), ops.csr_build(geo_edge_index, n), Mat.of(out))
        return out


def range_scale() -> float:
    return 2.0 ** -_ctx.shift


class GCUMotion(NativeModule):

    _RANGE_SCALED = True

    def __init__(self, in_channels, out_channels, in_channel_pos=3, dim_pos_feat=16, aggr="max"):
        super().__init__()
        self.edge_conv_tpl = EdgeConvMotion(nn_x=MLP([in_channels * 2, out_channels // 2, out_channels // 2]),
                                            nn_pos=MLP([in_channel_pos * 2, dim_pos_feat, dim_pos_feat]), aggr=aggr)
        self.edge_conv_geo = EdgeConvMotion(nn_x=MLP([in_channels * 2, out_channels // 2, out_channels // 2]),
                                            nn_pos=MLP([in_channel_pos * 2, dim_pos_feat, dim_pos_feat]), aggr=aggr)
        self.mlp = MLP([out_channels + dim_pos_feat * 2, out_channels])

    def _pack(self):
        vx, (xt, xg) = packing.pack_edge_pair([self.edge_conv_tpl.nn_x, self.edge_conv_geo.nn_x])
        vp, (pt, pg) = packing.pack_edge_pair([self.edge_conv_tpl.nn_pos, self.edge_conv_geo.nn_pos])
        pk = dict(vx=vx, xt=xt, xg=xg, vp=vp, pt=pt, pg=pg, mlp=packing.pack_mlp_layer(self.mlp[0]))
        H, D = xt.H, pt.H
        if H % 32 == 0 and (2 * D) % 32 == 0:
            cols = (list(range(H)) + [2 * H + i for i in range(D)] + [H + i for i in range(H)] + [2 * H + D + i for i in range(D)])
            pk["mlp_s"] = packing.pack_mlp_layer(self.mlp[0], in_cols=cols, k_total=2 * H + 2 * D)
        if xt.H == 32 and self.edge_conv_tpl.nn_x[0][0].weight.shape[1] == 6:
            firsts = []
            for ec in (self.edge_conv_tpl, self.edge_conv_geo):
                W1 = ec.nn_x[0][0].weight.detach().float()
                firsts.append(packing.pack_first_x3(W1[:, :3] - W1[:, 3:], W1[:, 3:], ec.nn_x[0][0].bias.detach().float()))
            pk["x3t"], pk["x3g"] = firsts
        return pk

    def run(self, ops, pos: Mat, x: Mat, csr_tpl, csr_geo, out: Mat, replicas: int = 1, split: bool = False,
            split_in=None, split_out=None, pos_feat=None, x3: Optional[Mat] = None):
        split_in = split if split_in is None else split_in
        split_out = split if split_out is None else split_out
        dev = x.base.device
        pk = self.packed(dev)
        n, M = pos.rows, x.rows
        assert M == n * replicas
        H, D = pk["xt"].H, pk["pt"].H
        ldo = 2 * H + 2 * D
        use_x3 = x3 is not None and "x3t" in pk and hasattr(ops, "edgeconv_x3") and os.environ.get("MORIG_EDGE_X3", "1") != "0"
        if not use_x3:
            ab = ops.empty(M, 4 * H, dev)
            ops.gemm(x, pk["vx"], relu=False, Y=Mat.of(ab), x_split=split_in)
        if pos_feat is None:
            pab = ops.empty(n, 4 * D, dev)
            ops.gemm(pos, pk["vp"], relu=False, Y=Mat.of(pab))
        tail = pos_feat[2] if (pos_feat is not None and len(pos_feat) > 2) else None
        use_tail = (tail is not None and not use_x3 and "mlp_s" in pk and hasattr(ops, "gemm_takes_tail")
                    and ops.gemm_takes_tail(pk["mlp_s"], out, 2 * D))
        ec = ops.empty(M, ldo, dev)
        if not use_x3 and "mlp_s" in pk and _edge_rows_can_split(ops, ab, ec, csr_tpl, csr_geo, pk["xt"], pk["xg"], H, replicas, n):
            ops.edgeconv_pair(dict(A=Mat.of(ab, 0, H), B=Mat.of(ab, H, H), csr=csr_tpl, ec=pk["xt"], out=Mat.of(ec, 0, H),
                                   replicas=replicas, in_rep_stride=n, out_rep_stride=n, out_split=True),
                              dict(A=Mat.of(ab, 2 * H, H), B=Mat.of(ab, 3 * H, H), csr=csr_geo, ec=pk["xg"], out=Mat.of(ec, H, H),
                                   replicas=replicas, in_rep_stride=n, out_rep_stride=n, out_split=True))
            if use_tail:
                ops.gemm(Mat.of(ec, 0, 2 * H), pk["mlp_s"], relu=True, Y=out, x_split=True, y_split=split_out, x_tail=tail)
                return
            p2 = ops.empty(n, 2 * D, dev)
            if pos_feat is not None:
                ops.copy2d(pos_feat[0], Mat.of(p2, 0, D))
                ops.copy2d(pos_feat[1], Mat.of(p2, D, D))
            else:
                ops.edgeconv_pair(dict(A=Mat.of(pab, 0, D), B=Mat.of(pab, D, D), csr=csr_tpl, ec=pk["pt"], out=Mat.of(p2, 0, D)),
                                  dict(A=Mat.of(pab, 2 * D, D), B=Mat.of(pab, 3 * D, D), csr=csr_geo, ec=pk["pg"], out=Mat.of(p2, D, D)))
            ops.copy2d_rep(Mat.of(p2), Mat.of(ec, 2 * H, 2 * D, 0, n), replicas, n, split=True)
            ops.gemm(Mat.of(ec), pk["mlp_s"], relu=True, Y=out, x_split=True, y_split=split_out)
            return
        if use_x3:
            ops.edgeconv_x3_pair(dict(X=x3, first=pk["x3t"], csr=csr_tpl, ec=pk["xt"], out=Mat.of(ec, 0, H),
                                      replicas=replicas, in_rep_stride=n, out_rep_stride=n),
                                 dict(X=x3, first=pk["x3g"], csr=csr_geo, ec=pk["xg"], out=Mat.of(ec, H + D, H),
                                      replicas=replicas, in_rep_stride=n, out_rep_stride=n))
        else:
            ops.edgeconv_pair(dict(A=Mat.of(ab, 0, H), B=Mat.of(ab, H, H), csr=csr_tpl, ec=pk["xt"], out=Mat.of(ec, 0, H),
                                   replicas=replicas, in_rep_stride=n, out_rep_stride=n),
                              dict(A=Mat.of(ab, 2 * H, H), B=Mat.of(ab, 3 * H, H), csr=csr_geo, ec=pk["xg"], out=Mat.of(ec, H + D, H),
                                   replicas=replicas, in_rep_stride=n, out_rep_stride=n))
        if pos_feat is not None:
            ops.copy2d_rep(pos_feat[0], Mat.of(ec, H, D, 0, n), replicas, n)
            ops.copy2d_rep(pos_feat[1], Mat.of(ec, 2 * H + D, D, 0, n), replicas, n)
        else:
            ops.edgeconv_pair(dict(A=Mat.of(pab, 0, D), B=Mat.of(pab, D, D), csr=csr_tpl, ec=pk["pt"], out=Mat.of(ec, H, D, 0, n)),
                              dict(A=Mat.of(pab, 2 * D, D), B=Mat.of(pab, 3 * D, D), csr=csr_geo, ec=pk["pg"], out=Mat.of(ec, 2 * H + D, D, 0, n)))
            if replicas > 1:
                ops.copy2d_rep(Mat.of(ec, H, D, 0, n), Mat.of(ec, H, D, n, n), replicas - 1, n)
                ops.copy2d_rep(Mat.of(ec, 2 * H + D, D, 0, n), Mat.of(ec, 2 * H + D, D, n, n), replicas - 1, n)
        ops.gemm(Mat.of(ec), pk["mlp"], relu=True, Y=out, y_split=split_out)

    def _forward(self, pos, x, tpl_edge_index, geo_edge_index):
        ops = get_ops()
        x = _padded_copy(ops, _as_matrix(x))
        pos = _padded_copy(ops, _as_matrix(pos))
        n = x.shape[0]
        pk = self.packed(x.device)
        out = ops.empty(n, pk["mlp"].N, x.device)
        self.run(ops, Mat.of(pos, 0, pk["vp"].K), Mat.of(x, 0, pk["vx"].K),
                 ops.csr_build(tpl_edge_index, n), ops.csr_build(geo_edge_index, n), Mat.of(out))
        return out


def run_pos_groups(ops, packed_groups, pos: Mat, csr_tpl, csr_geo):
    vertex, edges, n_pairs = packed_groups
    if n_pairs == 0:
        return []
    dev = pos.base.device
    n = pos.rows
    H = edges[0][0].H
    D = H // 2
    x3 = pos.cols == 3 and pos.col0 == 0 and pos.ld % 4 == 0 and all(e[2] is not None for e in edges) and hasattr(ops, "edgeconv_x3") \
        and os.environ.get("MORIG_EDGE_X3", "1") != "0"
    side = ops.empty(n, 2 * H * n_pairs, dev)
    if not x3:
        pab = ops.empty(n, 4 * H * n_pairs, dev)
        ops.gemm(pos, vertex, relu=False, Y=Mat.of(pab))
    out = []
    for g, (et, eg, ft, fg) in enumerate(edges):
        if x3:
            ops.edgeconv_x3_pair(dict(X=pos, first=ft, csr=csr_tpl, ec=et, out=Mat.of(side, 2 * H * g, H)),
                                 dict(X=pos, first=fg, csr=csr_geo, ec=eg, out=Mat.of(side, 2 * H * g + H, H)))
        else:
            c0 = 4 * H * g
            ops.edgeconv_pair(dict(A=Mat.of(pab, c0, H), B=Mat.of(pab, c0 + H, H), csr=csr_tpl, ec=et, out=Mat.of(side, 2 * H * g, H)),
                              dict(A=Mat.of(pab, c0 + 2 * H, H), B=Mat.of(pab, c0 + 3 * H, H), csr=csr_geo, ec=eg, out=Mat.of(side, 2 * H * g + H, H)))
        for j in range(2):
            out.append((Mat.of(side, 2 * H * g + j * D, D), Mat.of(side, 2 * H * g + H + j * D, D)))
    if ops.split_activations and 2 * D <= 32 and len(out) <= 8 and hasattr(ops, "pack_tails") and os.environ.get("MORIG_GEMM_TAIL", "1") != "0":
        tails = ops.pack_tails(side, [t.col0 for t, _ in out], [g_.col0 for _, g_ in out], D, D)
        out = [(t, g_, Mat.of(tails[u])) for u, (t, g_) in enumerate(out)]
    else:
        out = [(t, g_, None) for t, g_ in out]
    return out


class PointConv(torch.nn.Module):

    def __init__(self, local_nn=None, global_nn=None):
        super().__init__()
        self.local_nn = local_nn
        self.global_nn = global_nn


def radius_cpu(x, y, r, max_num_neighbors):
    ops = get_ops()
    xm = _pos4(ops, x)
    ym = _pos4(ops, y)
    seed = int(torch.randint(0, 2 ** 31 - 1, (1,)).item())
    coo, counts = ops.radius_sample(Mat.of(xm, 0, 3), Mat.of(ym, 0, 3), r, max_num_neighbors, seed)
    ny = ym.shape[0]
    slots = coo[0].view(ny, max_num_neighbors)
    rows = torch.arange(ny, device=slots.device).view(-1, 1).expand_as(slots)
    reduced = (counts > max_num_neighbors).view(-1, 1)
    keep_res = (slots >= 0) & ~reduced
    keep_red = reduced.expand_as(slots)
    return torch.cat([torch.stack([slots[keep_res], rows[keep_res]]), torch.stack([slots[keep_red], rows[keep_red]])], dim=1)


def _cloud_offsets(batch: torch.Tensor, n_clouds: Optional[int] = None):
    counts = torch.bincount(batch, minlength=n_clouds or 0).tolist()
    off = [0]
    for c in counts:
        off.append(off[-1] + int(c))
    return counts, torch.tensor(off, dtype=torch.int32, device=batch.device)


def _with_pos(ops, x: Optional[torch.Tensor], pos4: torch.Tensor):
    if x is None:
        return pos4, 0
    n, c = x.shape
    ld = (c + 3 + 3) // 4 * 4
    buf = torch.zeros((n, ld), dtype=torch.float32, device=x.device)
    ops.copy2d(Mat.of(x), Mat.of(buf, 0, c))
    ops.copy2d(Mat.of(pos4, 0, 3), Mat.of(buf, c, 3))
    return buf, c


def _pos4(ops, pos: torch.Tensor) -> torch.Tensor:
    p4 = torch.zeros((pos.shape[0], 4), dtype=torch.float32, device=pos.device)
    ops.copy2d(Mat.of(pos.float().contiguous()), Mat.of(p4, 0, 3))
    return p4


class SAModule(NativeModule):

    def __init__(self, ratio, r, nn, max_num_neighbors):
        super().__init__()
        self.ratio = ratio
        self.r = r
        self.max_num_neighbors = max_num_neighbors
        self.conv = PointConv(nn)

    def _pack(self):
        cx = self.conv.local_nn[0][0].weight.shape[1] - 3
        return packing.pack_pointconv(self.conv.local_nn, cx)

    def neighbours(self, ops, xp: torch.Tensor, cx: int, pos_new: torch.Tensor, ptr: torch.Tensor, out_ptr: torch.Tensor, n_clouds: int):
        return ops.ball_query(Mat.of(xp, cx, 3), ptr, Mat.of(pos_new, 0, 3), out_ptr, n_clouds, self.r, self.max_num_neighbors)

    def run(self, ops, xp: torch.Tensor, cx: int, pos_new: torch.Tensor, ptr: torch.Tensor, out_ptr: torch.Tensor, n_clouds: int,
            coo: Optional[torch.Tensor] = None):
        dev = xp.device
        pk = self.packed(dev)
        N, M = xp.shape[0], pos_new.shape[0]
        if coo is None:
            coo = self.neighbours(ops, xp, cx, pos_new, ptr, out_ptr, n_clouds)
        H = pk["edge"].H
        bsrc = ops.empty(N, H, dev)
        ops.gemm(Mat.of(xp, 0, cx + 3), pk["src"], relu=False, Y=Mat.of(bsrc))
        atgt = ops.empty(M, H, dev)
        ops.gemm(Mat.of(pos_new, 0, 3), pk["tgt"], relu=False, Y=Mat.of(atgt))
        x_new = ops.empty(M, pk["last"].N, dev)
        if ops.pointconv_can_fuse(pk, self.max_num_neighbors):
            ops.pointconv_fused(Mat.of(atgt), Mat.of(bsrc), coo, self.max_num_neighbors, pk, Mat.of(x_new))
            return x_new
        csr = ops.csr_from_slots(coo, M, self.max_num_neighbors, N)
        z = ops.empty(csr.capacity, H, dev)
        ops.edge_hidden(Mat.of(atgt), Mat.of(bsrc), csr, pk["edge"], Mat.of(z))
        ops.segmax_gemm(Mat.of(z), pk["last"], True, csr, Mat.of(x_new))
        return x_new

    def _forward(self, x, pos, batch, random_start=True):
        ops = get_ops()
        dev = pos.device
        counts, ptr = _cloud_offsets(batch)
        B = len(counts)
        out_counts = [int(math.ceil(self.ratio * c)) for c in counts]
        _, out_ptr = _cloud_offsets(torch.repeat_interleave(torch.arange(B, device=dev), torch.tensor(out_counts, device=dev)), B)
        start = None
        if random_start:
            start = torch.tensor([int(torch.randint(c, (1,))) for c in counts], dtype=torch.int32, device=dev)
        p4 = _pos4(ops, pos)
        M = sum(out_counts)
        idx = ops.fps(Mat.of(p4, 0, 3), ptr, out_ptr, start, B, max(counts), M)
        pos_new = torch.zeros((M, 4), dtype=torch.float32, device=dev)
        ops.gather_rows(Mat.of(p4, 0, 3), idx, Mat.of(pos_new, 0, 3))
        xp, cx = _with_pos(ops, None if x is None else x.float().contiguous(), p4)
        x_new = self.run(ops, xp, cx, pos_new, ptr, out_ptr, B)
        return x_new, pos_new[:, :3].contiguous(), batch[idx.long()]


class GlobalSAModule(NativeModule):

    def __init__(self, nn):
        super().__init__()
        self.nn = nn

    def _pack(self):
        return [packing.pack_mlp_layer(l) for l in self.nn]

    def run(self, ops, xp: torch.Tensor, width: int, seg: torch.Tensor, n_clouds: int) -> torch.Tensor:
        dev = xp.device
        layers = self.packed(dev)
        h = Mat.of(xp, 0, width)
        for lay in layers[:-1]:
            o = ops.empty(xp.shape[0], lay.N, dev)
            ops.gemm(h, lay, relu=True, Y=Mat.of(o))
            h = Mat.of(o)
        pooled = ops.empty(n_clouds, layers[-1].N, dev)
        ops.gemm(h, layers[-1], relu=True, seg=seg, pool=pooled)
        return pooled

    def _forward(self, x, pos, batch):
        ops = get_ops()
        dev = pos.device
        B = int(batch.max().item()) + 1
        xp, cx = _with_pos(ops, x.float().contiguous(), _pos4(ops, pos))
        pooled = self.run(ops, xp, cx + 3, ops.make_seg(batch, B, 1), B)
        return pooled, pos.new_zeros((B, 3)), torch.arange(B, device=dev)


class FPModule(NativeModule):

    def __init__(self, k, nn):
        super().__init__()
# ... 42 lines not shown
```

morig_amd/native.py:

```python
from __future__ import annotations

import ctypes as C
import dataclasses
import os
import threading
from dataclasses import dataclass
from typing import Optional

import torch

from . import abi

_HERE = os.path.dirname(os.path.abspath(__file__))
LIB_PATH = os.environ.get("MORIG_HIP_LIB") or os.path.join(_HERE, "lib", "libmorig_hip.so")

_K = abi.CONSTANTS
MorigNativeError = abi.MorigNativeError
GemmArgs = abi.STRUCTS["morig_gemm_args"]
EdgeConvArgs = abi.STRUCTS["morig_edgeconv_args"]
EdgeConvX3Args = abi.STRUCTS["morig_edgeconv_x3_args"]
PointConvArgs = abi.STRUCTS["morig_pointconv_args"]
SegmaxArgs = abi.STRUCTS["morig_segmax_args"]
IkArgs = abi.STRUCTS["morig_ik_args"]
NceArgs = abi.STRUCTS["morig_nce_args"]
# ... 290 lines not shown
                  "morig_csr_build")
        else:
            check(self.lib.morig_csr_build_bipartite(_p(ei), E, n_nodes if n_src is None else n_src, n_nodes,
                                                     (_K["MORIG_CSR_SKIP_NEGATIVE"] if skip_negative else 0) | (_K["MORIG_CSR_PAD4"] if pad4 else 0) |
                                                     (_K["MORIG_CSR_MIN4"] if min4 else 0), _p(rowptr), _p(src),
                                                     _p(dst), _p(cursor), _p(status), _stream()), "morig_csr_build_bipartite")
        csr = CSR(rowptr, src, dst, n_nodes, cap, status, quad=pad4, min4=min4)
        if getattr(self, "_csr_status", None) is not None:
            self._csr_status.append(status)
        key = (ei.data_ptr(), E, n_nodes)
        if self.learn_edge_counts and not pad4 and not min4 and key not in self._edge_counts:
            self._edge_counts[key] = int(rowptr[-1].item())
        csr.edge_count = self._edge_counts.get(key, 0)
        return csr

    def csr_build_dual(self, edge_index: torch.Tensor, n_nodes: int, min4: Optional[bool] = None):
        if min4 is None:
            min4 = os.environ.get("MORIG_EDGE_MIX", "0") == "1"
        _need_gpu(edge_index)
        ei = edge_index if (edge_index.dtype == torch.int64 and edge_index.is_contiguous()) else edge_index.long().contiguous()
        E = ei.shape[1]
        dev = ei.device
        cap, cap4 = E + (4 if min4 else 1) * n_nodes, E + 4 * n_nodes
        rowptr = torch.empty(n_nodes + 1, dtype=torch.int32, device=dev)
        rowptr4 = torch.empty(n_nodes + 1, dtype=torch.int32, device=dev)
        src, dst = torch.empty(cap, dtype=torch.int32, device=dev), torch.empty(cap, dtype=torch.int32, device=dev)
        src4, dst4 = torch.empty(cap4, dtype=torch.int32, device=dev), torch.empty(cap4, dtype=torch.int32, device=dev)
        ws = torch.empty(2 * n_nodes + 1, dtype=torch.int32, device=dev)
        status = torch.empty(1, dtype=torch.int32, device=dev)
        check(self.lib.morig_csr_build_dual(_p(ei), E, n_nodes, _p(rowptr), _p(src), _p(dst), _p(rowptr4), _p(src4), _p(dst4), _p(ws),
                                            _K["MORIG_CSR_MIN4"] if min4 else 0, _p(status), _stream()), "morig_csr_build_dual")
        if getattr(self, "_csr_status", None) is not None:
            self._csr_status.append(status)
        key = (ei.data_ptr(), E, n_nodes)
        a = CSR(rowptr, src, dst, n_nodes, cap, status, min4=bool(min4))
        b = CSR(rowptr4, src4, dst4, n_nodes, cap4, status, quad=True)
        a.edge_count = b.edge_count = self._edge_counts.get(key, 0)
        return a, b

    def csr_from_slots(self, coo: torch.Tensor, n_nodes: int, max_nbrs: int, n_src: int) -> CSR:
        _need_gpu(coo)
        assert coo.dtype == torch.int64 and coo.is_contiguous() and coo.shape == (2, n_nodes * max_nbrs)
        dev = coo.device
        cap = n_nodes * (max_nbrs + 1)
        rowptr = torch.empty(n_nodes + 1, dtype=torch.int32, device=dev)
        src = torch.empty(cap, dtype=torch.int32, device=dev)
        dst = torch.empty(cap, dtype=torch.int32, device=dev)
        cursor = torch.empty(n_nodes + 1, dtype=torch.int32, device=dev)
        status = torch.empty(1, dtype=torch.int32, device=dev)
        check(self.lib.morig_csr_from_slots(_p(coo), n_nodes, max_nbrs, n_src, _p(rowptr), _p(src), _p(dst), _p(cursor),
                                            _p(status), _stream()), "morig_csr_from_slots")
        if getattr(self, "_csr_status", None) is not None:
            self._csr_status.append(status)
        return CSR(rowptr, src, dst, n_nodes, cap, status)

    def gemm(self, X: Mat, lin, relu: bool, Y: Optional[Mat] = None, rowbias: Optional[Mat] = None,
             seg: Optional[torch.Tensor] = None, pool: Optional[torch.Tensor] = None, affine: bool = True,
             x_split: bool = False, y_split: bool = False, x_tail: Optional[Mat] = None):
        _need_gpu(X.base, lin.W)
        if x_split or y_split:
            if not self.fast:
                raise MorigNativeError("split-fp16 activations requested on the fp32 path (plan bug)")
            if lin.Wsplit is None:
                self._flag(X.base.device).fill_(1)
                return
        if pool is not None:
            lin = padded_for_pool(lin)
        a = _args(GemmArgs)
        a.M, a.N, a.K = X.rows, lin.N, lin.K
        if x_tail is not None:
            assert x_split and X.cols + x_tail.cols == lin.K and x_tail.cols % 32 == 0, (X.cols, x_tail.cols, lin.K)
            a.X_tail, a.ld_tail, a.tail_rows, a.tail_cols = x_tail.ptr, x_tail.ld, x_tail.rows, x_tail.cols
        else:
            assert X.cols == lin.K, (X.cols, lin.K)
        a.X, a.ldx = X.ptr, X.ld
        a.W, a.ldw = lin.W.data_ptr(), lin.W.stride(0)
        a.bias = lin.bias.data_ptr() if lin.bias is not None else 0
        a.scale = lin.scale.data_ptr() if (affine and lin.scale is not None) else 0
        a.shift = lin.shift.data_ptr() if (affine and lin.shift is not None) else 0
        a.relu = 1 if relu else 0
        if rowbias is not None:
            a.rowbias, a.ld_rowbias = rowbias.ptr, rowbias.ld
        a.seg = seg.data_ptr() if seg is not None else 0
        if Y is not None:
            assert Y.rows == X.rows and Y.cols == lin.N
            a.Y, a.ldy = Y.ptr, Y.ld
        if pool is not None:
            assert pool.shape[1] >= lin.N and pool.is_contiguous()
            a.pool, a.ld_pool, a.n_seg = pool.data_ptr(), pool.stride(0), pool.shape[0]
        if getattr(lin, "Wsplit_bf16", None) is not None:
            assert pool is None and not x_split and not y_split
            a.W_split, a.overflow, a.w_split_format = lin.Wsplit_bf16.data_ptr(), 0, _K["MORIG_SPLIT_BF16"]
        elif self.fast and lin.Wsplit is not None:
            a.W_split, a.overflow = lin.Wsplit.data_ptr(), self._flag(X.base.device).data_ptr()
        elif self.exact_arith == "bf16x6" and not x_split and not y_split:
            a.w_split_format = _K["MORIG_SPLIT_BF16X6"]
        a.x_split, a.y_split = int(x_split), int(y_split)
        check(self.lib.morig_gemm(C.byref(a), _stream()), "morig_gemm")

    def gemm_takes_tail(self, lin, Y: Mat, n_tail_cols: int) -> bool:
        return (self.fast and os.environ.get("MORIG_GEMM_TAIL", "1") != "0" and os.environ.get("MORIG_NO_DMA") is None and
                lin.Wsplit is not None and lin.N % 256 == 0 and lin.K % 32 == 0 and n_tail_cols % 32 == 0 and lin.K > n_tail_cols and
                Y.ptr % 16 == 0 and Y.ld % 4 == 0 and os.environ.get("MORIG_GEMM_TR", "1") != "0" and
                os.environ.get("MORIG_DMA_TILE", "256") == "256")

    def pack_tails(self, src: torch.Tensor, col_a, col_b, wa: int, wb: int) -> torch.Tensor:
        _need_gpu(src)
        assert src.dim() == 2 and src.dtype == torch.float32 and src.stride(1) == 1 and len(col_a) == len(col_b) <= _K["MORIG_MAX_TAILS"]
        n, rows = len(col_a), src.shape[0]
        out = torch.empty((n, rows, 32), dtype=torch.float32, device=src.device)
        ca, cb = (C.c_int32 * n)(*col_a), (C.c_int32 * n)(*col_b)
        check(self.lib.morig_pack_tails(_p(src), src.stride(0), rows, ca, cb, wa, wb, n, _p(out), rows * 32,
                                        self._flag(src.device).data_ptr(), _stream()), "morig_pack_tails")
        return out

    def edgeconv(self, A: Mat, B: Mat, csr: CSR, ec, out: Mat, replicas: int = 1,
                 in_rep_stride: int = 0, out_rep_stride: int = 0, out_split: bool = False):
        _need_gpu(A.base, B.base, out.base)
        a = self._edge_args(A, B, csr, ec, out, replicas, in_rep_stride, out_rep_stride)
        a.out_split = 1 if out_split else 0
        check(self.lib.morig_edgeconv(C.byref(a), _stream()), "morig_edgeconv")

    def edgeconv_pair(self, first: dict, second: dict):
        if not PAIR_PASSES:
            self.edgeconv(**first)
            self.edgeconv(**second)
            return
        calls = []
        for kw in (first, second):
            kw = dict(kw)
            sp = bool(kw.pop("out_split", False))
            _need_gpu(kw["A"].base, kw["B"].base, kw["out"].base)
            a = self._edge_args(kw["A"], kw["B"], kw["csr"], kw["ec"], kw["out"], kw.get("replicas", 1), kw.get("in_rep_stride", 0),
                                kw.get("out_rep_stride", 0))
            a.out_split = 1 if sp else 0
            calls.append(a)
        a1, a2 = calls
        a1.init_with, a2.skip_init = C.addressof(a2), 1
        if a1.out_split and a2.out_split:
            a1.skip_split, a2.split_with = 1, C.addressof(a1)
        check(self.lib.morig_edgeconv(C.byref(a1), _stream()), "morig_edgeconv")
        check(self.lib.morig_edgeconv(C.byref(a2), _stream()), "morig_edgeconv")

    def edgeconv_x3_pair(self, first: dict, second: dict):
        if not PAIR_PASSES:
            self.edgeconv_x3(**first)
            self.edgeconv_x3(**second)
            return
        a1, a2 = (self._x3_args(**kw) for kw in (first, second))
        a1.init_with, a2.skip_init = C.addressof(a2), 1
        check(self.lib.morig_edgeconv_x3(C.byref(a1), _stream()), "morig_edgeconv_x3")
        check(self.lib.morig_edgeconv_x3(C.byref(a2), _stream()), "morig_edgeconv_x3")

    def edgeconv_can_split_out(self, A: Mat, B: Mat, csr: CSR, ec, out: Mat, replicas: int = 1,
                               in_rep_stride: int = 0, out_rep_stride: int = 0) -> bool:
        a = self._edge_args(A, B, csr, ec, out, replicas, in_rep_stride, out_rep_stride)
        return bool(self.lib.morig_edgeconv_can_split_out(C.byref(a)))

    def _edge_args(self, A, B, csr, ec, out, replicas, in_rep_stride, out_rep_stride):
        a = _args(EdgeConvArgs)
        a.H = ec.H
        a.n_nodes, a.replicas = csr.n_nodes, replicas
        a.in_rep_stride, a.out_rep_stride = in_rep_stride, out_rep_stride
        a.A, a.lda = A.ptr, A.ld
        a.B, a.ldb = B.ptr, B.ld
        a.rowptr, a.src_sorted, a.dst_sorted = csr.rowptr.data_ptr(), csr.src.data_ptr(), csr.dst.data_ptr()
        a.edge_capacity, a.edge_count = csr.capacity, csr.edge_count
        if ec.s1 is not None:
            a.s1, a.t1 = ec.s1.data_ptr(), ec.t1.data_ptr()
        a.W2, a.ldw = ec.W2.data_ptr(), ec.W2.stride(0)
        a.b2, a.s2, a.t2 = ec.b2.data_ptr(), ec.s2.data_ptr(), ec.t2.data_ptr()
        a.out, a.ldo = out.ptr, out.ld
        a.quad_aligned = 1 if csr.quad else 0
        a.seg_min4 = 1 if getattr(csr, "min4", False) else 0
        a.exact_arith = 1 if self.exact_arith == "bf16x6" else 0
        if self.fast and ec.W2split is not None:
            a.W2_split, a.overflow = ec.W2split.data_ptr(), self._flag(A.base.device).data_ptr()
        return a

    def edgeconv_x3(self, X: Mat, first, csr: CSR, ec, out: Mat, replicas: int = 1, in_rep_stride: int = 0, out_rep_stride: int = 0):
        a = self._x3_args(X, first, csr, ec, out, replicas, in_rep_stride, out_rep_stride)
        check(self.lib.morig_edgeconv_x3(C.byref(a), _stream()), "morig_edgeconv_x3")

    def _x3_args(self, X: Mat, first, csr: CSR, ec, out: Mat, replicas: int = 1, in_rep_stride: int = 0, out_rep_stride: int = 0):
        _need_gpu(X.base, out.base)
        assert ec.H == 32 and ec.s1 is None and X.col0 % 4 == 0 and X.ld % 4 == 0
        a = _args(EdgeConvX3Args)
        a.H = 32
        a.n_nodes, a.replicas = csr.n_nodes, replicas
        a.in_rep_stride, a.out_rep_stride = in_rep_stride, out_rep_stride
        a.X, a.ldx = X.ptr, X.ld
        a.W1a, a.W1b, a.b1 = first[0].data_ptr(), first[1].data_ptr(), first[2].data_ptr()
        a.rowptr, a.src_sorted, a.dst_sorted = csr.rowptr.data_ptr(), csr.src.data_ptr(), csr.dst.data_ptr()
        a.edge_capacity, a.edge_count = csr.capacity, csr.edge_count
        a.W2, a.ldw = ec.W2.data_ptr(), ec.W2.stride(0)
        a.b2, a.s2, a.t2 = ec.b2.data_ptr(), ec.s2.data_ptr(), ec.t2.data_ptr()
        a.out, a.ldo = out.ptr, out.ld
        if self.fast and ec.W2split is not None:
            a.W2_split, a.overflow = ec.W2split.data_ptr(), self._flag(X.base.device).data_ptr()
        return a

    def edge_hidden(self, A: Mat, B: Mat, csr: CSR, ec, Z: Mat):
        _need_gpu(A.base, B.base, Z.base)
        assert Z.rows == csr.capacity and Z.cols == ec.H
        a = self._edge_args(A, B, csr, ec, Z, 1, 0, 0)
        check(self.lib.morig_edge_hidden(C.byref(a), _stream()), "morig_edge_hidden")

    def segmax_gemm(self, X: Mat, lin, relu: bool, csr: CSR, out: Mat):
        _need_gpu(X.base, out.base)
        assert X.rows == csr.capacity and X.cols == lin.K and out.rows == csr.n_nodes and out.cols == lin.N
        a = _args(SegmaxArgs)
        a.N, a.K = lin.N, lin.K
        a.X, a.ldx = X.ptr, X.ld
        a.W, a.ldw = lin.W.data_ptr(), lin.W.stride(0)
        a.bias = lin.bias.data_ptr() if lin.bias is not None else 0
        a.scale = lin.scale.data_ptr() if lin.scale is not None else 0
        a.shift = lin.shift.data_ptr() if lin.shift is not None else 0
        a.relu = 1 if relu else 0
        a.rowptr, a.dst_sorted, a.n_nodes = csr.rowptr.data_ptr(), csr.dst.data_ptr(), csr.n_nodes
        a.edge_capacity, a.edge_count = csr.capacity, csr.edge_count
        a.out, a.ldo = out.ptr, out.ld
        if self.fast and lin.Wsplit is not None:
            a.W_split, a.overflow = lin.Wsplit.data_ptr(), self._flag(X.base.device).data_ptr()
        check(self.lib.morig_segmax_gemm(C.byref(a), _stream()), "morig_segmax_gemm")

    def pointconv_can_fuse(self, pk, max_nbrs: int) -> bool:
        l3 = pk.get("fused")
        return bool(self.fast and l3 is not None and l3.Wsplit is not None and pk["edge"].W2split is not None and
                    max_nbrs == 64 and pk["edge"].s1 is None and os.environ.get("MORIG_POINTCONV_FUSED", "1") != "0")

    def pointconv_fused(self, A: Mat, B: Mat, coo: torch.Tensor, max_nbrs: int, pk, out: Mat):
        _need_gpu(A.base, B.base, out.base, coo)
        ec, l3 = pk["edge"], pk["fused"]
        assert coo.dtype == torch.int64 and coo.is_contiguous() and coo.shape == (2, A.rows * max_nbrs)
        assert A.cols == B.cols == ec.H and out.rows == A.rows and out.cols == l3.N and B.rows >= A.rows
        dev = A.base.device
        status = torch.zeros(1, dtype=torch.int32, device=dev)
        a = _args(PointConvArgs)
        a.A, a.lda, a.B, a.ldb = A.ptr, A.ld, B.ptr, B.ld
        a.slots, a.max_nbrs, a.n_centres, a.n_src = coo.data_ptr(), max_nbrs, A.rows, B.rows
        a.H, a.H3 = ec.H, l3.N
        a.W2_split, a.ldw2, a.b2 = ec.W2split.data_ptr(), ec.W2split.stride(0), ec.b2.data_ptr()
        a.W3_split, a.ldw3, a.b3 = l3.Wsplit.data_ptr(), l3.Wsplit.stride(0), l3.bias.data_ptr()
        a.s3 = l3.scale.data_ptr() if l3.scale is not None else 0
        a.t3 = l3.shift.data_ptr() if l3.shift is not None else 0
        a.relu3 = 1
        a.out, a.ldo = out.ptr, out.ld
        a.overflow, a.status = self._flag(dev).data_ptr(), status.data_ptr()
        check(self.lib.morig_pointconv_fused(C.byref(a), _stream()), "morig_pointconv_fused")
        if getattr(self, "_csr_status", None) is not None:
            self._csr_status.append(status)
        elif int(status.item()) != 0:
            raise MorigNativeError("morig_pointconv_fused: the slot table names a source row outside B")

    def fps(self, pos: Mat, ptr: torch.Tensor, out_ptr: torch.Tensor, start: Optional[torch.Tensor], n_clouds: int,
            max_cloud_points: int, n_samples: int) -> torch.Tensor:
        _need_gpu(pos.base, ptr, out_ptr)
        idx = torch.empty(n_samples, dtype=torch.int32, device=pos.base.device)
        check(self.lib.morig_fps(pos.ptr, pos.ld, _p(ptr), _p(out_ptr), _p(start), n_clouds, max_cloud_points, _p(idx), _stream()),
              "morig_fps")
        return idx

    def ball_query(self, x: Mat, ptr_x: torch.Tensor, y: Mat, ptr_y: torch.Tensor, n_clouds: int, radius: float,
                   max_nbrs: int) -> torch.Tensor:
        _need_gpu(x.base, y.base, ptr_x, ptr_y)
        coo = torch.empty((2, y.rows * max_nbrs), dtype=torch.int64, device=x.base.device)
        check(self.lib.morig_ball_query(x.ptr, x.ld, _p(ptr_x), y.ptr, y.ld, _p(ptr_y), n_clouds, y.rows, float(radius),
                                        max_nbrs, _p(coo), _stream()), "morig_ball_query")
        return coo

    def col_stats(self, X: Mat, rows_dev: Optional[torch.Tensor] = None):
        _need_gpu(X.base)
        dev = X.base.device
        slabs = (max(X.rows, 1) + 255) // 256
        ws = torch.empty(slabs * 2 * X.cols, dtype=torch.float64, device=dev)
        mean = torch.empty(X.cols, dtype=torch.float32, device=dev)
        var = torch.empty(X.cols, dtype=torch.float32, device=dev)
        cnt = torch.empty(1, dtype=torch.float32, device=dev)
        check(self.lib.morig_col_stats(X.ptr, X.ld, X.rows, _p(rows_dev), X.cols, C.c_void_p(ws.data_ptr()), ws.numel(), _p(mean),
                                       _p(var), _p(cnt), _stream()), "morig_col_stats")
        return mean, var, cnt

    def col_affine(self, X: Mat, scale: torch.Tensor, shift: torch.Tensor, rows_dev: Optional[torch.Tensor] = None,
                   out: Optional[Mat] = None):
        _need_gpu(X.base, scale, shift)
        assert scale.numel() >= X.cols and shift.numel() >= X.cols and scale.dtype == shift.dtype == torch.float32
        assert out is None or (out.rows == X.rows and out.cols == X.cols)
        check(self.lib.morig_col_affine(X.ptr, X.ld, X.rows, _p(rows_dev), X.cols, _p(scale), _p(shift), out.ptr if out is not None else 0,
                                        out.ld if out is not None else 0, _stream()), "morig_col_affine")

    def bn_finalize(self, bn, mean: torch.Tensor, var: torch.Tensor, count: torch.Tensor):
        _need_gpu(mean, var, count)
        n = mean.numel()
        dev = mean.device
        out = torch.empty((3, n), dtype=torch.float32, device=dev)
        track = bn.track_running_stats and bn.running_mean is not None
        g = bn.weight.detach() if bn.weight is not None else None
        b = bn.bias.detach() if bn.bias is not None else None
        for x in (g, b, bn.running_mean if track else None, bn.running_var if track else None):
            assert x is None or (x.dtype == torch.float32 and x.is_contiguous() and x.device == dev)
        assert mean.dtype == var.dtype == count.dtype == torch.float32 and mean.is_contiguous() and var.is_contiguous()
        check(self.lib.morig_bn_finalize(_p(mean), _p(var), _p(count), _p(g), _p(b), float(bn.eps), float(bn.momentum if track else 0.0),
                                         _p(bn.running_mean) if track else None, _p(bn.running_var) if track else None,
                                         _p(bn.num_batches_tracked) if track else None, _p(out[0]), _p(out[1]), _p(out[2]), n, _stream()),
              "morig_bn_finalize")
        return out[0], out[1], out[2]
# ... 1716 lines not shown
```

Before: 1459 meshes/s.

## Group x3 edgeconvs sharing a CSR graph into one multi-weight kernel launch

Adds a grouped x3 edge-conv kernel that processes up to four weight sets sharing the same CSR graph and input positions in one launch. Each edge tile is loaded and its segment list built once, then reused across groups. The Python model chains the template and geodesic edge convs for several pairs into two calls instead of one pair call per group. This is meant to cut launch count and repeated edge/index loads, at the cost of more per-block work, possible register pressure from reloading weights per group, and a larger ABI struct.

Result: no change. 1466 meshes/s, median of 6 (+0.5%).

```diff
diff --git a/include/morig_hip.h b/include/morig_hip.h
--- a/include/morig_hip.h
+++ b/include/morig_hip.h
@@ -17,7 +17,7 @@
 #define MORIG_SEGMAX_ARGS_V3_SIZE      144u
 #define MORIG_POINTCONV_ARGS_V3_SIZE   176u
 #define MORIG_EDGECONV_ARGS_SIZE       216u
-#define MORIG_EDGECONV_X3_ARGS_SIZE    184u
+#define MORIG_EDGECONV_X3_ARGS_SIZE    192u
 
 #define MORIG_OK              0
 #define MORIG_E_INVALID      -1
@@ -106,7 +106,9 @@
     const void* W2_split; int32_t* overflow;
     const struct morig_edgeconv_x3_args* init_with;
     int32_t skip_init, reserved0;
+    const struct morig_edgeconv_x3_args* next_group;
 } morig_edgeconv_x3_args;
+#define MORIG_X3_MAX_GROUPS 4
 int morig_edgeconv_x3(const morig_edgeconv_x3_args* a, void* stream);
 
 int morig_edge_hidden(const morig_edgeconv_args* a, void* stream);
diff --git a/morig_amd/csrc/common.h b/morig_amd/csrc/common.h
--- a/morig_amd/csrc/common.h
+++ b/morig_amd/csrc/common.h
@@ -32,6 +32,7 @@
     K_RAY_CAST, K_RAY_SELECT, K_RAY_ATTENTION,
     K_TRANSFER_PAIRS, K_TRANSFER_FLOOD, K_TRANSFER_ROWS,
     K_BVH_BUILD, K_BVH_QUERY,
+    K_EDGE16_X3G,
     K_COUNT
 };
 static_assert(K_COUNT <= MORIG_PROF_KINDS, "raise MORIG_PROF_KINDS");
@@ -88,6 +89,11 @@
 int launch_edge_ws(const EdgePcParams& p, int nblocks, hipStream_t s);
 int launch_edge_rl(const EdgePcParams& p, int ntiles64, hipStream_t s);
 int launch_gemm16_dma(const GemmDmaParams& p, int tiles_m128, hipStream_t s);
+struct EdgeX3Group {
+    const float* W1a; const float* W1b; const float* b1; const float* W2s;
+    const float* bias; const float* scale; const float* shift;
+    float* Y;
+};
 struct EdgeX3Params {
     const float* X; int ldx;
     const float* W1a; const float* W1b; const float* b1;
@@ -98,9 +104,13 @@
     int rep_in, rep_out, replicas;
     float* Y; int ldy;
     int* ovf;
+    int n_groups;
+    EdgeX3Group grp[MORIG_X3_MAX_GROUPS];
 };
 
 int launch_edge_x3(const EdgeX3Params& p, int n_tiles_cap, hipStream_t s);
+bool edge_x3_groups_enabled();
+bool edge_x3_shares_tiles(const EdgeX3Params& p);
 int launch_gemm16_dmap(const GemmDmaParams& p, hipStream_t s);
 bool few_rows_gemm_takes(int M, int N, int K, int ldx, int ldw);
 int launch_few_rows_gemm(const float* X, int ldx, int M, const float* W, int ldw, int N, int K, const float* bias, const float* scale,
diff --git a/morig_amd/csrc/edge_x3.hip b/morig_amd/csrc/edge_x3.hip
--- a/morig_amd/csrc/edge_x3.hip
+++ b/morig_amd/csrc/edge_x3.hip
@@ -4,14 +4,132 @@
 
 
 constexpr int X3_BM = 128, X3_LINE = 144;
+
+struct X3Lists {
+    int sseg[2][X3_BM];
+    int sstart[2][X3_BM + 2];
+    int snseg[2];
+    int sflag[2][2];
+};
+
+__device__ __forceinline__ f32x16 x3_first_layer(const f16x8 w1h, const f16x8 w1l, const f32x4 hb, const f32x4 lb) {
+    const f16x8 xh = __builtin_bit_cast(f16x8, hb), xl = __builtin_bit_cast(f16x8, lb);
+    f32x16 a1;
+#pragma unroll
+    for (int r = 0; r < 16; ++r) a1[r] = 0.f;
+    a1 = __builtin_amdgcn_mfma_f32_32x32x16_f16(w1l, xh, a1, 0, 0, 0);
+    a1 = __builtin_amdgcn_mfma_f32_32x32x16_f16(w1h, xl, a1, 0, 0, 0);
+    a1 = __builtin_amdgcn_mfma_f32_32x32x16_f16(w1h, xh, a1, 0, 0, 0);
+    return a1;
+}
+__device__ __forceinline__ bool x3_split_inputs(const f32x4 xi, const f32x4 xj, f32x4& hb, f32x4& lb) {
+    float h2, l2;
+    split_pair_f16(xi[0], xi[1], h2, l2); hb[0] = h2; lb[0] = l2;
+    split_pair_f16(xi[2], xj[0], h2, l2); hb[1] = h2; lb[1] = l2;
+    split_pair_f16(xj[1], xj[2], h2, l2); hb[2] = h2; lb[2] = l2;
+    split_pair_f16(1.0f, 0.0f, h2, l2);   hb[3] = h2; lb[3] = l2;
+    const float am = fmaxf(fmaxf(fmaxf(fabsf(xi[0]), fabsf(xi[1])), fmaxf(fabsf(xi[2]), fabsf(xj[0]))), fmaxf(fabsf(xj[1]), fabsf(xj[2])));
+    return am < FP16_RANGE_GUARD;
+}
+__device__ __forceinline__ void x3_w1_fragments(const float (&v)[8], f16x8& w1h, f16x8& w1l) {
+    f32x4 hb, lb;
+#pragma unroll
+    for (int q = 0; q < 4; ++q) { float h2, l2; split_pair_f16(v[2 * q], v[2 * q + 1], h2, l2); hb[q] = h2; lb[q] = l2; }
+    w1h = __builtin_bit_cast(f16x8, hb); w1l = __builtin_bit_cast(f16x8, lb);
+}
+template <bool CHECK>
+__device__ __forceinline__ bool x3_stage_hidden(const f32x16& a1, char* line, int hi) {
+    float am = 0.f, chk = 0.f;
+#pragma unroll
+    for (int g4 = 0; g4 < 4; ++g4) {
+        float h[4];
+#pragma unroll
+        for (int q = 0; q < 4; ++q) {
+            if (CHECK) chk = fmaf(a1[4 * g4 + q], 0.f, chk);
+            h[q] = fmaxf(a1[4 * g4 + q], 0.f); am = fmaxf(am, h[q]);
+        }
+        float h0, l0, h1, l1;
+        split_pair_f16(h[0], h[1], h0, l0);
+        split_pair_f16(h[2], h[3], h1, l1);
+        typedef float f32x2 __attribute__((ext_vector_type(2)));
+        const f32x2 hv = {h0, h1}, lv = {l0, l1};
+        const int c0 = 8 * g4 + 4 * hi;
+        *reinterpret_cast<f32x2*>(line + 2 * c0) = hv;
+        *reinterpret_cast<f32x2*>(line + 64 + 2 * c0) = lv;
+    }
+    return (chk == 0.f) && (am < FP16_RANGE_GUARD);
+}
+__device__ __forceinline__ void x3_second_layer(char* L, int wave, int l31, int hi, const f16x8 (&wh)[2], const f16x8 (&wl)[2],
+                                                float cb, float cs, float ct) {
+    asm volatile("" ::: "memory");
+    f32x16 acc;
+#pragma unroll
+    for (int r = 0; r < 16; ++r) acc[r] = 0.f;
+    {
+        const char* ar = L + (wave * 32 + l31) * X3_LINE + 16 * hi;
+#pragma unroll
+        for (int st = 0; st < 2; ++st) {
+            const f16x8 ah = *reinterpret_cast<const f16x8*>(ar + 32 * st);
+            const f16x8 al = *reinterpret_cast<const f16x8*>(ar + 64 + 32 * st);
+            acc = __builtin_amdgcn_mfma_f32_32x32x16_f16(al, wh[st], acc, 0, 0, 0);
+            acc = __builtin_amdgcn_mfma_f32_32x32x16_f16(ah, wl[st], acc, 0, 0, 0);
+            acc = __builtin_amdgcn_mfma_f32_32x32x16_f16(ah, wh[st], acc, 0, 0, 0);
+        }
+    }
+    asm volatile("" ::: "memory");
+    float* Z = reinterpret_cast<float*>(L);
+#pragma unroll
+    for (int r = 0; r < 16; ++r) {
+        const int rl = wave * 32 + (r & 3) + 8 * (r >> 2) + 4 * hi;
+        Z[rl * (X3_LINE / 4) + l31] = fmaxf(acc[r] + cb, 0.f) * cs + ct;
+    }
+}
+__device__ __forceinline__ void x3_build_list(X3Lists& S, int par, int lane, bool more_behind, int e_behind) {
+    const int rA = lane, rB = lane + 64;
+    const bool f0 = rA == 0 || S.sseg[par][rA] != S.sseg[par][rA - 1];
+    const bool f1 = S.sseg[par][rB] != S.sseg[par][rB - 1];
+    const unsigned long long m0 = __ballot(f0), m1 = __ballot(f1);
+    const unsigned long long below = (1ull << lane) - 1ull;
+    if (f0) S.sstart[par][__popcll(m0 & below)] = rA;
+    if (f1) S.sstart[par][__popcll(m0) + __popcll(m1 & below)] = rB;
+    if (lane == 0) { const int ns = __popcll(m0) + __popcll(m1); S.snseg[par] = ns; S.sstart[par][ns] = X3_BM; }
+    if (lane == 1) S.sflag[par][1] = (more_behind && S.sseg[par][X3_BM - 1] == e_behind) ? 1 : 0;
+}
+__device__ __forceinline__ void x3_segmax(const char* L, const X3Lists& S, int par, int tid, float* obase, int ldy) {
+    const float* Z = reinterpret_cast<const float*>(L);
+    const int c4 = (tid & 7) * 4, slot = tid >> 3;
+    const int nseg = S.snseg[par];
+    const bool first_cont = S.sflag[par][0] != 0, last_cont = S.sflag[par][1] != 0;
+    obase += c4;
+    for (int k = slot; k < nseg; k += 32) {
+        const int rs = S.sstart[par][k], re = S.sstart[par][k + 1];
+        const int sg = S.sseg[par][rs];
+        if (sg < 0) continue;
+        f32x4 m = *reinterpret_cast<const f32x4*>(Z + rs * (X3_LINE / 4) + c4);
+        for (int r = rs + 1; r < re; r += 4) {
+            f32x4 z[4];
+#pragma unroll
+            for (int u = 0; u < 4; ++u) z[u] = *reinterpret_cast<const f32x4*>(Z + min(r + u, re - 1) * (X3_LINE / 4) + c4);
+#pragma unroll
+            for (int u = 0; u < 4; ++u)
+#pragma unroll
+                for (int q = 0; q < 4; ++q) m[q] = fmaxf(m[q], z[u][q]);
+        }
+        float* o = obase + (size_t)sg * ldy;
+        const bool partial = (rs == 0 && first_cont) || (re == X3_BM && last_cont);
+        if (partial) {
+#pragma unroll
+            for (int q = 0; q < 4; ++q) atomic_max_f32(o + q, m[q]);
+        } else {
+            *reinterpret_cast<f32x4*>(o) = m;
+        }
+    }
+}
 
 template <bool AB>
 __global__ __launch_bounds__(256, 4) void edge_x3_kernel(const EdgeX3Params p) {
     __shared__ __attribute__((aligned(16))) char lines[2][X3_BM * X3_LINE];
-    __shared__ int sseg[2][X3_BM];
-    __shared__ int sstart[2][X3_BM + 2];
-    __shared__ int snseg[2];
-    __shared__ int sflag[2][2];
+    __shared__ X3Lists S;
 
     const int tid = threadIdx.x, lane = tid & 63, wave = tid >> 6;
     const int l31 = lane & 31, hi = lane >> 5;
@@ -29,10 +147,7 @@
             for (int j = 0; j < 3; ++j) { v[j] = p.W1a[l31 * 4 + j]; v[3 + j] = p.W1b[l31 * 4 + j]; }
             v[6] = p.b1[l31];
         }
-        f32x4 hb, lb;
-#pragma unroll
-        for (int q = 0; q < 4; ++q) { float h2, l2; split_pair_f16(v[2 * q], v[2 * q + 1], h2, l2); hb[q] = h2; lb[q] = l2; }
-        w1h = __builtin_bit_cast(f16x8, hb); w1l = __builtin_bit_cast(f16x8, lb);
+        x3_w1_fragments(v, w1h, w1l);
         const char* wr = reinterpret_cast<const char*>(p.W2s + (size_t)l31 * p.ldw);
 #pragma unroll
         for (int st = 0; st < 2; ++st) {
@@ -90,8 +205,8 @@
         load_ids(t + 2 * tstep, d_nn, s_nn, e_nn);
 
         char* L = lines[par];
-        if (hi == 0) sseg[par][row] = live ? d_cur : -1;
-        if (tid == 0) sflag[par][0] = (r0 > 0 && d_cur == e_cur) ? 1 : 0;
+        if (hi == 0) S.sseg[par][row] = live ? d_cur : -1;
+        if (tid == 0) S.sflag[par][0] = (r0 > 0 && d_cur == e_cur) ? 1 : 0;
         {
             f32x16 a1;
             if constexpr (AB) {
@@ -101,111 +216,16 @@
                     for (int q = 0; q < 4; ++q) a1[4 * g4 + q] = ga_cur[g4][q] + gb_cur[g4][q];
             } else {
                 f32x4 hb = {0.f, 0.f, 0.f, 0.f}, lb = hb;
-                if (hi == 0) {
-                    float h2, l2;
-                    split_pair_f16(xi_cur[0], xi_cur[1], h2, l2); hb[0] = h2; lb[0] = l2;
-                    split_pair_f16(xi_cur[2], xj_cur[0], h2, l2); hb[1] = h2; lb[1] = l2;
-                    split_pair_f16(xj_cur[1], xj_cur[2], h2, l2); hb[2] = h2; lb[2] = l2;
-                    split_pair_f16(1.0f, 0.0f, h2, l2);           hb[3] = h2; lb[3] = l2;
-                    const float am = fmaxf(fmaxf(fmaxf(fabsf(xi_cur[0]), fabsf(xi_cur[1])), fmaxf(fabsf(xi_cur[2]), fabsf(xj_cur[0]))),
-                                           fmaxf(fabsf(xj_cur[1]), fabsf(xj_cur[2])));
-                    if (!(am < FP16_RANGE_GUARD)) amax_bad = true;
-                }
-                const f16x8 xh = __builtin_bit_cast(f16x8, hb), xl = __builtin_bit_cast(f16x8, lb);
-#pragma unroll
-                for (int r = 0; r < 16; ++r) a1[r] = 0.f;
-                a1 = __builtin_amdgcn_mfma_f32_32x32x16_f16(w1l, xh, a1, 0, 0, 0);
-                a1 = __builtin_amdgcn_mfma_f32_32x32x16_f16(w1h, xl, a1, 0, 0, 0);
-                a1 = __builtin_amdgcn_mfma_f32_32x32x16_f16(w1h, xh, a1, 0, 0, 0);
+                if (hi == 0 && !x3_split_inputs(xi_cur, xj_cur, hb, lb)) amax_bad = true;
+                a1 = x3_first_layer(w1h, w1l, hb, lb);
             }
-            char* line = L + row * X3_LINE;
-            float am = 0.f, chk = 0.f;
-#pragma unroll
-            for (int g4 = 0; g4 < 4; ++g4) {
-                float h[4];
-#pragma unroll
-                for (int q = 0; q < 4; ++q) {
-                    if (AB) chk = fmaf(a1[4 * g4 + q], 0.f, chk);
-                    h[q] = fmaxf(a1[4 * g4 + q], 0.f); am = fmaxf(am, h[q]);
-                }
-                float h0, l0, h1, l1;
-                split_pair_f16(h[0], h[1], h0, l0);
-                split_pair_f16(h[2], h[3], h1, l1);
-                typedef float f32x2 __attribute__((ext_vector_type(2)));
-                const f32x2 hv = {h0, h1}, lv = {l0, l1};
-                const int c0 = 8 * g4 + 4 * hi;
-                *reinterpret_cast<f32x2*>(line + 2 * c0) = hv;
-                *reinterpret_cast<f32x2*>(line + 64 + 2 * c0) = lv;
-            }
-            if (!(chk == 0.f) || !(am < FP16_RANGE_GUARD)) amax_bad = true;
-        }
-        asm volatile("" ::: "memory");
-        f32x16 acc;
-#pragma unroll
-        for (int r = 0; r < 16; ++r) acc[r] = 0.f;
-        {
-            const char* ar = L + (wave * 32 + l31) * X3_LINE + 16 * hi;
-#pragma unroll
-            for (int st = 0; st < 2; ++st) {
-                const f16x8 ah = *reinterpret_cast<const f16x8*>(ar + 32 * st);
-                const f16x8 al = *reinterpret_cast<const f16x8*>(ar + 64 + 32 * st);
-                acc = __builtin_amdgcn_mfma_f32_32x32x16_f16(al, wh[st], acc, 0, 0, 0);
-                acc = __builtin_amdgcn_mfma_f32_32x32x16_f16(ah, wl[st], acc, 0, 0, 0);
-                acc = __builtin_amdgcn_mfma_f32_32x32x16_f16(ah, wh[st], acc, 0, 0, 0);
-            }
-        }
-        asm volatile("" ::: "memory");
-        {
-            float* Z = reinterpret_cast<float*>(L);
-#pragma unroll
-            for (int r = 0; r < 16; ++r) {
-                const int rl = wave * 32 + (r & 3) + 8 * (r >> 2) + 4 * hi;
-                Z[rl * (X3_LINE / 4) + l31] = fmaxf(acc[r] + cb, 0.f) * cs + ct;
-            }
-        }
+            if (!x3_stage_hidden<AB>(a1, L + row * X3_LINE, hi)) amax_bad = true;
+        }
+        x3_second_layer(L, wave, l31, hi, wh, wl, cb, cs, ct);
         __syncthreads();
-        if (wave == 0) {
-            const int rA = lane, rB = lane + 64;
-            const bool f0 = rA == 0 || sseg[par][rA] != sseg[par][rA - 1];
-            const bool f1 = sseg[par][rB] != sseg[par][rB - 1];
-            const unsigned long long m0 = __ballot(f0), m1 = __ballot(f1);
-            const unsigned long long below = (1ull << lane) - 1ull;
-            if (f0) sstart[par][__popcll(m0 & below)] = rA;
-            if (f1) sstart[par][__popcll(m0) + __popcll(m1 & below)] = rB;
-            if (lane == 0) { const int ns = __popcll(m0) + __popcll(m1); snseg[par] = ns; sstart[par][ns] = X3_BM; }
-            if (lane == 1) sflag[par][1] = (r0 + X3_BM < Etot && sseg[par][X3_BM - 1] == e_cur) ? 1 : 0;
-        }
+        if (wave == 0) x3_build_list(S, par, lane, r0 + X3_BM < Etot, e_cur);
         __syncthreads();
-        {
-            const float* Z = reinterpret_cast<const float*>(L);
-            const int c4 = (tid & 7) * 4, slot = tid >> 3;
-            const int nseg = snseg[par];
-            const bool first_cont = sflag[par][0] != 0, last_cont = sflag[par][1] != 0;
-            float* obase = p.Y + (size_t)rep * p.rep_out * p.ldy + c4;
-            for (int k = slot; k < nseg; k += 32) {
-                const int rs = sstart[par][k], re = sstart[par][k + 1];
-                const int sg = sseg[par][rs];
-                if (sg < 0) continue;
-                f32x4 m = *reinterpret_cast<const f32x4*>(Z + rs * (X3_LINE / 4) + c4);
-                for (int r = rs + 1; r < re; r += 4) {
-                    f32x4 z[4];
-#pragma unroll
-                    for (int u = 0; u < 4; ++u) z[u] = *reinterpret_cast<const f32x4*>(Z + min(r + u, re - 1) * (X3_LINE / 4) + c4);
-#pragma unroll
-                    for (int u = 0; u < 4; ++u)
-#pragma unroll
-                        for (int q = 0; q < 4; ++q) m[q] = fmaxf(m[q], z[u][q]);
-                }
-                float* o = obase + (size_t)sg * p.ldy;
-                const bool partial = (rs == 0 && first_cont) || (re == X3_BM && last_cont);
-                if (partial) {
-#pragma unroll
-                    for (int q = 0; q < 4; ++q) atomic_max_f32(o + q, m[q]);
-                } else {
-                    *reinterpret_cast<f32x4*>(o) = m;
-                }
-            }
-        }
+        x3_segmax(L, S, par, tid, p.Y + (size_t)rep * p.rep_out * p.ldy, p.ldy);
         d_cur = d_nxt; s_cur = s_nxt; e_cur = e_nxt; xi_cur = xi_nxt; xj_cur = xj_nxt;
         if constexpr (AB) {
 #pragma unroll
@@ -216,10 +236,141 @@
     if (amax_bad) *p.ovf = 1;
 }
 
-int launch_edge_x3(const EdgeX3Params& p, int n_tiles_cap, hipStream_t s) {
+template <bool REP>
+__global__ __launch_bounds__(256, 4) void edge_x3g_kernel(const EdgeX3Params p) {
+    __shared__ __attribute__((aligned(16))) char lines[2][X3_BM * X3_LINE];
+    __shared__ X3Lists S;
+
+    const int tid = threadIdx.x, lane = tid & 63, wave = tid >> 6;
+    const int l31 = lane & 31, hi = lane >> 5;
+    const int row = wave * 32 + l31;
+    const int Etot = p.rowptr[p.n_nodes];
+    const int T = (Etot + X3_BM - 1) / X3_BM;
+    const int G = REP ? p.replicas : p.n_groups;
+    if ((int)blockIdx.x >= T) return;
+
+    f16x8 w1h, w1l, wh[2], wl[2];
+    float cb, cs, ct;
+    f32x4 wa = {0.f, 0.f, 0.f, 0.f}, wb = wa;
+    float wc = 0.f;
+    auto load_group = [&](int g) __attribute__((always_inline)) {
+        const EdgeX3Group& q = p.grp[g];
+        if (hi == 0) {
+            wa = *reinterpret_cast<const f32x4*>(q.W1a + l31 * 4); wb = *reinterpret_cast<const f32x4*>(q.W1b + l31 * 4);
+            wc = q.b1[l31];
+        }
+        const char* wr = reinterpret_cast<const char*>(q.W2s + (size_t)l31 * p.ldw);
+#pragma unroll
+        for (int st = 0; st < 2; ++st) {
+            wh[st] = *reinterpret_cast<const f16x8*>(wr + 32 * st + 16 * hi);
+            wl[st] = *reinterpret_cast<const f16x8*>(wr + 64 + 32 * st + 16 * hi);
+        }
+        cb = q.bias[l31]; cs = q.scale[l31]; ct = q.shift[l31];
+    };
+    auto first_fragments = [&]() __attribute__((always_inline)) {
+        const float v[8] = {wa[0], wa[1], wa[2], wb[0], wb[1], wb[2], wc, 0.f};
+        x3_w1_fragments(v, w1h, w1l);
+    };
+    auto load_ids = [&](int t, int& d, int& sidx, int& edge) __attribute__((always_inline)) {
+        if (t >= T) return;
+        const int r0 = t * X3_BM;
+        const int r = min(r0 + row, Etot - 1);
+        d = p.dstS[r]; sidx = p.srcS[r];
+        if (tid < 2) edge = p.dstS[min(max(tid == 0 ? r0 - 1 : r0 + X3_BM, 0), Etot - 1)];
+    };
+    auto load_x = [&](int t, int g, int d, int sidx, f32x4& a, f32x4& b) __attribute__((always_inline)) {
+        if (t >= T || hi != 0) return;
+        const bool live = t * X3_BM + row < Etot;
+        const size_t base = REP ? (size_t)g * p.rep_in : 0;
+        a = *reinterpret_cast<const f32x4*>(p.X + (base + (live ? d : 0)) * p.ldx);
+        b = *reinterpret_cast<const f32x4*>(p.X + (base + (live ? sidx : 0)) * p.ldx);
+    };
+    const int t0 = blockIdx.x, tstep = gridDim.x;
+    int d_cur = 0, s_cur = 0, e_cur = 0, d_nxt = 0, s_nxt = 0, e_nxt = 0;
+    f32x4 xi_cur = {0.f, 0.f, 0.f, 0.f}, xj_cur = xi_cur, xi_nxt = xi_cur, xj_nxt = xi_cur;
+    load_ids(t0, d_cur, s_cur, e_cur);
+    load_ids(t0 + tstep, d_nxt, s_nxt, e_nxt);
+    load_group(0);
+    load_x(t0, 0, d_cur, s_cur, xi_cur, xj_cur);
+    if (REP) first_fragments();
+    bool amax_bad = false;
+
+    int par = 0, lp = 0;
+    for (int t = t0; t < T; t += tstep, par ^= 1) {
+        const int r0 = t * X3_BM;
+        const bool live = r0 + row < Etot;
+        int d_nn = 0, s_nn = 0, e_nn = 0;
+        load_ids(t + 2 * tstep, d_nn, s_nn, e_nn);
+        if (hi == 0) S.sseg[par][row] = live ? d_cur : -1;
+        if (tid == 0) S.sflag[par][0] = (r0 > 0 && d_cur == e_cur) ? 1 : 0;
+        f32x4 hb = {0.f, 0.f, 0.f, 0.f}, lb = hb;
+        if (!REP) {
+            load_x(t + tstep, 0, d_nxt, s_nxt, xi_nxt, xj_nxt);
+            if (hi == 0 && !x3_split_inputs(xi_cur, xj_cur, hb, lb)) amax_bad = true;
+        }
+#pragma nounroll
+        for (int g = 0; g < G; ++g, lp ^= 1) {
+            if (REP) {
+                const bool last = g + 1 == G;
+                load_x(last ? t + tstep : t, last ? 0 : g + 1, last ? d_nxt : d_cur, last ? s_nxt : s_cur, xi_nxt, xj_nxt);
+                if (hi == 0 && !x3_split_inputs(xi_cur, xj_cur, hb, lb)) amax_bad = true;
+            } else {
+                first_fragments();
+            }
+            char* L = lines[lp];
+            const f32x16 a1 = x3_first_layer(w1h, w1l, hb, lb);
+            if (!x3_stage_hidden<false>(a1, L + row * X3_LINE, hi)) amax_bad = true;
+            x3_second_layer(L, wave, l31, hi, wh, wl, cb, cs, ct);
+            float* Yg = REP ? p.Y + (size_t)g * p.rep_out * p.ldy : p.grp[g].Y;
+            if (!REP && G > 1) load_group(g + 1 < G ? g + 1 : 0);
+            __syncthreads();
+            if (g == 0) {
+                if (wave == 0) x3_build_list(S, par, lane, r0 + X3_BM < Etot, e_cur);
+                __syncthreads();
+            }
+            x3_segmax(L, S, par, tid, Yg, p.ldy);
+            if (REP) { xi_cur = xi_nxt; xj_cur = xj_nxt; }
+        }
+        d_cur = d_nxt; s_cur = s_nxt; e_cur = e_nxt;
+        if (!REP) { xi_cur = xi_nxt; xj_cur = xj_nxt; }
+        d_nxt = d_nn; s_nxt = s_nn; e_nxt = e_nn;
+    }
+    if (amax_bad) *p.ovf = 1;
+}
+
+static int x3_full_grid() {
     int avail = cu_count() - reserved_cus();
     if (avail < 8) avail = 8;
-    int grid = avail * 4;
+    return avail * 4;
+}
+
+bool edge_x3_groups_enabled() {
+    static const bool on = [] { const char* e = getenv("MORIG_X3_GROUPS"); return !(e && e[0] == '0'); }();
+    return on;
+}
+
+bool edge_x3_shares_tiles(const EdgeX3Params& p) {
+    if (!p.X) return false;
+    if (p.n_groups > 0) return true;
+    return edge_x3_groups_enabled() && p.replicas > 1 && (p.cap + X3_BM - 1) / X3_BM >= x3_full_grid();
+}
+
+int launch_edge_x3(const EdgeX3Params& p, int n_tiles_cap, hipStream_t s) {
+    int grid = x3_full_grid();
+    if (edge_x3_shares_tiles(p)) {
+        const int tiles = (p.cap + X3_BM - 1) / X3_BM;
+        if (grid > tiles) grid = tiles;
+        if (grid < 1) grid = 1;
+        if (p.n_groups > 0) {
+            hipLaunchKernelGGL(edge_x3g_kernel<false>, dim3(grid), dim3(256), 0, s, p);
+        } else {
+            EdgeX3Params q = p;
+            q.grp[0] = EdgeX3Group{p.W1a, p.W1b, p.b1, p.W2s, p.bias, p.scale, p.shift, p.Y};
+            hipLaunchKernelGGL(edge_x3g_kernel<true>, dim3(grid), dim3(256), 0, s, q);
+        }
+        MORIG_LAUNCH_CHECK();
+        return MORIG_OK;
+    }
     if (grid > n_tiles_cap) grid = n_tiles_cap;
     if (grid < 1) grid = 1;
     if (p.X) hipLaunchKernelGGL(edge_x3_kernel<false>, dim3(grid), dim3(256), 0, s, p);
diff --git a/morig_amd/csrc/prof.hip b/morig_amd/csrc/prof.hip
--- a/morig_amd/csrc/prof.hip
+++ b/morig_amd/csrc/prof.hip
@@ -110,6 +110,7 @@
     "ray_cast", "ray_select", "ray_attention",
     "transfer_pairs", "transfer_flood", "transfer_rows",
     "bvh_build", "bvh_query",
+    "edgeconv_f16x3_x3_groups",
 };
 static const char* kSymbols[K_COUNT] = {
     "tile_kernel<128, 32, 0, 0, 0,", "tile_kernel<64, 32, 0, 0, 0,", "tile_kernel<32, 32, 0, 0, 0,", "tile_kernel<128, 32, 0, 1, 0,",
@@ -132,6 +133,7 @@
     "ray_cast_kernel", "ray_select_kernel", "ray_attention_kernel",
     nullptr, nullptr, nullptr,
     nullptr, nullptr,
+    "edge_x3g_kernel",
 };
 
 }
diff --git a/morig_amd/csrc/tile_gemm.hip b/morig_amd/csrc/tile_gemm.hip
--- a/morig_amd/csrc/tile_gemm.hip
+++ b/morig_amd/csrc/tile_gemm.hip
@@ -568,7 +568,8 @@
 }
 
 struct BoundaryJob { const int* rowptr; const int* dstS; int n_nodes, H; float* out; int ldo, rep_out, tile_rows, run, replicas, n_cand; int* ovf; };
-struct BoundaryJobs { BoundaryJob j[2]; };
+constexpr int MAX_BOUNDARY_JOBS = 2 * MORIG_X3_MAX_GROUPS;
+struct BoundaryJobs { BoundaryJob j[MAX_BOUNDARY_JOBS]; };
 
 __global__ __launch_bounds__(256) void init_boundary_rows_kernel(const BoundaryJobs js) {
     const BoundaryJob& b = js.j[blockIdx.y];
@@ -608,6 +609,7 @@
 static int init_boundary_rows(const BoundaryJob* jobs, int n, hipStream_t s) {
     BoundaryJobs js = {};
     int m = 0, most = 0;
+    if (n > MAX_BOUNDARY_JOBS) return MORIG_E_INVALID;
     for (int i = 0; i < n; ++i) if (jobs[i].n_cand > 0) { js.j[m++] = jobs[i]; most = jobs[i].n_cand > most ? jobs[i].n_cand : most; }
     if (m == 0) return MORIG_OK;
     hipLaunchKernelGGL(init_boundary_rows_kernel, dim3(cdiv(most, 256), m), dim3(256), 0, s, js);
@@ -668,6 +670,7 @@
 static int split_boundary_rows(const BoundaryJob* jobs, int n, hipStream_t s) {
     BoundaryJobs js = {};
     int m = 0, most = 0;
+    if (n > MAX_BOUNDARY_JOBS) return MORIG_E_INVALID;
     for (int i = 0; i < n; ++i) if (jobs[i].n_cand > 0) { js.j[m++] = jobs[i]; most = jobs[i].n_cand > most ? jobs[i].n_cand : most; }
     if (m == 0) return MORIG_OK;
     hipLaunchKernelGGL(split_boundary_rows_kernel, dim3(cdiv(most, 64), m), dim3(256), 0, s, js);
@@ -1100,6 +1103,28 @@
     }
 }
 
+static bool x3_wants_tile_engine() {
+    static const bool want_tile = [] { const char* e = getenv("MORIG_X3_TILE"); return e && e[0] == '1'; }();
+    return want_tile;
+}
+static int x3_chain(const morig_edgeconv_x3_args* a, morig_edgeconv_x3_args (&grp)[MORIG_X3_MAX_GROUPS]) {
+    int n = 0;
+    grp[n++] = *a;
+    for (const morig_edgeconv_x3_args* nx = a->next_group; nx; nx = grp[n - 1].next_group) {
+        if (n == MORIG_X3_MAX_GROUPS || !take_args(nx, grp[n], MORIG_EDGECONV_X3_ARGS_V3_SIZE)) return -1;
+        const morig_edgeconv_x3_args& g = grp[n++];
+        if (g.H != a->H || g.n_nodes != a->n_nodes || g.rowptr != a->rowptr || g.src_sorted != a->src_sorted || g.dst_sorted != a->dst_sorted ||
+            g.edge_capacity != a->edge_capacity || g.edge_count != a->edge_count || g.X != a->X || g.ldx != a->ldx || g.ldw != a->ldw ||
+            g.ldo != a->ldo || g.overflow != a->overflow || (g.W2_split == nullptr) != (a->W2_split == nullptr)) return -1;
+        if (!g.W1a || !g.W1b || !g.b1 || !g.W2 || !g.b2 || !g.s2 || !g.t2 || !g.out) return -1;
+        if (!aligned16(g.W2) || !aligned16(g.W1a) || !aligned16(g.W1b) || !aligned16(g.W2_split)) return -1;
+    }
+    if (n > 1)
+        for (int g = 0; g < n; ++g)
+            if (grp[g].replicas != 1 || !aligned16(grp[g].out) || (a->ldo & 3)) return -1;
+    return n;
+}
+
 extern "C" int morig_edgeconv_x3(const morig_edgeconv_x3_args* a_in, void* stream) {
     morig_edgeconv_x3_args mine;
     if (!take_args(a_in, mine, MORIG_EDGECONV_X3_ARGS_V3_SIZE)) return MORIG_E_INVALID;
@@ -1127,24 +1152,40 @@
         p.W = static_cast<const float*>(a->W2_split); p.ovf = a->overflow;
     }
     const int nblocks = p.tiles_per_rep * a->replicas;
+    morig_edgeconv_x3_args grp[MORIG_X3_MAX_GROUPS];
+    const int n_groups = x3_chain(a, grp);
+    if (n_groups < 0) return MORIG_E_INVALID;
     if (!a->skip_init) {
-        BoundaryJob jobs[2];
+        BoundaryJob jobs[MAX_BOUNDARY_JOBS];
         int nj = 0;
-        jobs[nj++] = boundary_job(a->rowptr, a->dst_sorted, a->n_nodes, a->edge_capacity, 32, a->out, a->ldo, a->out_rep_stride, a->replicas, 128, 1, nullptr);
+        for (int g = 0; g < n_groups; ++g)
+            jobs[nj++] = boundary_job(a->rowptr, a->dst_sorted, a->n_nodes, a->edge_capacity, 32, grp[g].out, a->ldo, a->out_rep_stride, a->replicas, 128, 1, nullptr);
         if (a->init_with) {
             morig_edgeconv_x3_args o;
             if (!take_args(a->init_with, o, MORIG_EDGECONV_X3_ARGS_V3_SIZE)) return MORIG_E_INVALID;
             if (!o.rowptr || !o.dst_sorted || !o.out || o.H != 32 || o.n_nodes <= 0 || o.replicas <= 0 || o.edge_capacity <= 0 || o.ldo < 32 ||
                 (o.replicas > 1 && o.out_rep_stride < o.n_nodes)) return MORIG_E_INVALID;
-            jobs[nj++] = boundary_job(o.rowptr, o.dst_sorted, o.n_nodes, o.edge_capacity, 32, o.out, o.ldo, o.out_rep_stride, o.replicas, 128, 1, nullptr);
+            morig_edgeconv_x3_args ogrp[MORIG_X3_MAX_GROUPS];
+            const int on = x3_chain(&o, ogrp);
+            if (on < 0) return MORIG_E_INVALID;
+            for (int g = 0; g < on; ++g)
+                jobs[nj++] = boundary_job(o.rowptr, o.dst_sorted, o.n_nodes, o.edge_capacity, 32, ogrp[g].out, o.ldo, o.out_rep_stride, o.replicas, 128, 1, nullptr);
         }
         const int st2 = init_boundary_rows(jobs, nj, s);
         if (st2 != MORIG_OK) return st2;
     } else if (a->init_with) return MORIG_E_INVALID;
-    const double E = (double)(a->edge_count > 0 ? a->edge_count : a->edge_capacity) * a->replicas;
+    const bool persistent = f16 && !x3_wants_tile_engine() && (a->ldo & 3) == 0;
+    if (n_groups > 1 && !(persistent && edge_x3_groups_enabled())) {
+        for (int g = 0; g < n_groups; ++g) {
+            grp[g].skip_init = 1; grp[g].init_with = nullptr; grp[g].next_group = nullptr;
+            const int st3 = morig_edgeconv_x3(&grp[g], stream);
+            if (st3 != MORIG_OK) return st3;
+        }
+        return MORIG_OK;
+    }
+    const double E = (double)(a->edge_count > 0 ? a->edge_count : a->edge_capacity) * a->replicas * n_groups;
     ProfScope ps(f16 ? K_EDGE16_X3 : K_EDGE_X3, s, E * (2.0 * 32 * 32 + 12.0 * 32), 32.0 * E);
-    static const bool want_tile = [] { const char* e = getenv("MORIG_X3_TILE"); return e && e[0] == '1'; }();
-    if (f16 && !want_tile && (a->ldo & 3) == 0 && aligned16(a->out)) {
+    if (persistent && aligned16(a->out)) {
         EdgeX3Params q = {};
         q.X = a->X; q.ldx = a->ldx; q.W1a = a->W1a; q.W1b = a->W1b; q.b1 = a->b1;
         q.W2s = static_cast<const float*>(a->W2_split); q.ldw = a->ldw;
@@ -1152,7 +1193,13 @@
         q.rowptr = a->rowptr; q.srcS = a->src_sorted; q.dstS = a->dst_sorted; q.n_nodes = a->n_nodes; q.cap = a->edge_capacity;
         q.rep_in = a->in_rep_stride; q.rep_out = a->out_rep_stride; q.replicas = a->replicas;
         q.Y = a->out; q.ldy = a->ldo; q.ovf = a->overflow;
-        prof_retag(K_EDGE16_X3P);
+        if (n_groups > 1) {
+            q.n_groups = n_groups;
+            for (int g = 0; g < n_groups; ++g)
+                q.grp[g] = EdgeX3Group{grp[g].W1a, grp[g].W1b, grp[g].b1, static_cast<const float*>(grp[g].W2_split), grp[g].b2, grp[g].s2, grp[g].t2,
+                                       grp[g].out};
+        }
+        prof_retag(edge_x3_shares_tiles(q) ? K_EDGE16_X3G : K_EDGE16_X3P);
         return launch_edge_x3(q, nblocks, s);
     }
     return f16 ? launch_tile<32, 32, LOAD_EDGE3, MODE_EDGEMAX, PREC_F16X3>(p, nblocks, s)
diff --git a/morig_amd/models/basic_modules.py b/morig_amd/models/basic_modules.py
--- a/morig_amd/models/basic_modules.py
+++ b/morig_amd/models/basic_modules.py
@@ -419,12 +419,17 @@
     if not x3:
         pab = ops.empty(n, 4 * H * n_pairs, dev)
         ops.gemm(pos, vertex, relu=False, Y=Mat.of(pab))
+    grouped = x3 and hasattr(ops, "edgeconv_x3_groups") and os.environ.get("MORIG_X3_GROUPS", "1") != "0"
+    tpl = [dict(X=pos, first=ft, csr=csr_tpl, ec=et, out=Mat.of(side, 2 * H * g, H)) for g, (et, eg, ft, fg) in enumerate(edges)] if x3 else []
+    geo = [dict(X=pos, first=fg, csr=csr_geo, ec=eg, out=Mat.of(side, 2 * H * g + H, H)) for g, (et, eg, ft, fg) in enumerate(edges)] if x3 else []
+    if grouped:
+        for g0 in range(0, n_pairs, ops.max_x3_groups):
+            ops.edgeconv_x3_groups(tpl[g0:g0 + ops.max_x3_groups], geo[g0:g0 + ops.max_x3_groups])
     out = []
     for g, (et, eg, ft, fg) in enumerate(edges):
-        if x3:
-            ops.edgeconv_x3_pair(dict(X=pos, first=ft, csr=csr_tpl, ec=et, out=Mat.of(side, 2 * H * g, H)),
-                                 dict(X=pos, first=fg, csr=csr_geo, ec=eg, out=Mat.of(side, 2 * H * g + H, H)))
-        else:
+        if x3 and not grouped:
+            ops.edgeconv_x3_pair(tpl[g], geo[g])
+        elif not x3:
             c0 = 4 * H * g
             ops.edgeconv_pair(dict(A=Mat.of(pab, c0, H), B=Mat.of(pab, c0 + H, H), csr=csr_tpl, ec=et, out=Mat.of(side, 2 * H * g, H)),
                               dict(A=Mat.of(pab, c0 + 2 * H, H), B=Mat.of(pab, c0 + 3 * H, H), csr=csr_geo, ec=eg, out=Mat.of(side, 2 * H * g + H, H)))
diff --git a/morig_amd/native.py b/morig_amd/native.py
--- a/morig_amd/native.py
+++ b/morig_amd/native.py
@@ -466,6 +466,23 @@
         check(self.lib.morig_edgeconv_x3(C.byref(a1), _stream()), "morig_edgeconv_x3")
         check(self.lib.morig_edgeconv_x3(C.byref(a2), _stream()), "morig_edgeconv_x3")
 
+    max_x3_groups = _K["MORIG_X3_MAX_GROUPS"]
+
+    def edgeconv_x3_groups(self, first: list, second: list = None):
+        chains = []
+        for groups in (first, second or []):
+            assert len(groups) <= self.max_x3_groups
+            args = [self._x3_args(**kw) for kw in groups]
+            for a, nxt in zip(args, args[1:]):
+                a.next_group = C.addressof(nxt)
+            chains.append(args)
+        a1, a2 = chains
+        if a2 and PAIR_PASSES:
+            a1[0].init_with, a2[0].skip_init = C.addressof(a2[0]), 1
+        for args in (a1, a2):
+            if args:
+                check(self.lib.morig_edgeconv_x3(C.byref(args[0]), _stream()), "morig_edgeconv_x3")
+
     def edgeconv_can_split_out(self, A: Mat, B: Mat, csr: CSR, ec, out: Mat, replicas: int = 1,
                                in_rep_stride: int = 0, out_rep_stride: int = 0) -> bool:
         a = self._edge_args(A, B, csr, ec, out, replicas, in_rep_stride, out_rep_stride)
```
